# revollllt/FP8_quantization

Hardware: AMD Instinct MI355X
Metric: ImageNet val images/sec, ResNet-18 FP8 approx_v9 (higher is better)
Workload: dtype fp32; 1 GPU; resnet18 E4M3 approx_v9 forward (dnsmp_factor=3, withComp=False, with_s2nn2s_opt, quant_btw_mult_accu, res_quantizer, fixed ranges), ImageNet-shaped synthetic batch, random-init weights with BN statistics estimated on 4 synthetic batches; global_batch=1024, per_gpu_batch=1024, approx_macs_per_image=1814073344, parallelism=dp1

## Files before the change

### fp8_quantization_amd/_lib.py

```python
import ctypes
import os

import torch

HERE = os.path.dirname(os.path.abspath(__file__))
LIB_PATH = os.environ.get("FP8A_LIB_PATH") or os.path.join(HERE, "lib", "libfp8approx.so")

APPROX, S2N, QBMA, GCLIP, TB = 1, 2, 4, 8, 16
V5, OFUF, OF_OPT, UF_OPT = 32, 64, 128, 256
OK, EINVAL, EFORMAT, EHIP = 0, -1, -2, -3
DENSE_E4M3, DENSE_E5M2, DENSE_BF16 = 0, 1, 2

SYMBOLS = ("fp8a_version", "fp8a_last_error", "fp8a_fallback_stats", "fp8a_path_stats", "fp8a_kernel_timing", "fp8a_kernel_time", "fp8a_set_option", "fp8a_decompose", "fp8a_quant", "fp8a_matmul_workspace_size",
           "fp8a_matmul_workspace_size_mnk", "fp8a_matmul", "fp8a_terms", "fp8a_conv2d_workspace_size", "fp8a_conv2d",
           "fp8a_conv2d_bn_act", "fp8a_conv2d_qin_workspace_size", "fp8a_conv2d_qin",
           "fp8a_conv2d_block_workspace_size", "fp8a_conv2d_block", "fp8a_max_pool2d", "fp8a_avg_pool2d_plane", "fp8a_im2col",
           "fp8a_fp8_quantize", "fp8a_matmul_qamaa", "fp8a_conv2d_qamaa", "fp8a_matmul_block_workspace_size",
           "fp8a_matmul_block", "fp8a_dense_matmul_workspace_size", "fp8a_dense_matmul",
           "fp8a_dense_conv2d_workspace_size", "fp8a_dense_conv2d", "fp8a_grouped_conv2d", "fp8a_dense_conv2d_fused", "fp8a_dense_stats", "fp8a_clock_stats",
           "fp8a_word_image_bytes", "fp8a_word_image_init", "fp8a_conv2d_chain", "fp8a_conv2d_wants_image",
           "fp8a_flag_arena_slot_bytes")

_lib = None


class NativeLibraryMissing(RuntimeError):
    pass


def load():
    global _lib
    if _lib is not None:
        return _lib
    if not os.path.exists(LIB_PATH):
        raise NativeLibraryMissing(
            f"{LIB_PATH} not found: build it with `python -m fp8_quantization_amd.build_native` "
            "(there is no CPU fallback for the approx-FP8 path)")
    L = ctypes.CDLL(LIB_PATH)
    P, I, I64, U, SZ = ctypes.c_void_p, ctypes.c_int, ctypes.c_int64, ctypes.c_uint32, ctypes.c_size_t
    F = ctypes.c_float
    sig = {
        "fp8a_version": ([], ctypes.c_char_p),
        "fp8a_last_error": ([], ctypes.c_char_p),
        "fp8a_fallback_stats": ([P, I], I),
        "fp8a_path_stats": ([P, I], I),
        "fp8a_kernel_timing": ([I], I),
        "fp8a_kernel_time": ([P, I], I),
        "fp8a_set_option": ([ctypes.c_char_p, I], I),
        "fp8a_decompose": ([P, I64, I64, I64, I, I, P, I64, U, P, P, P], I),
        "fp8a_quant": ([P, I64, I, I, P, U, P, P], I),
        "fp8a_matmul_workspace_size": ([], SZ),
        "fp8a_matmul_workspace_size_mnk": ([I64, I64, I64], SZ),
        "fp8a_matmul": ([P, I64, P, I64, I64, P, I64, I64, I64, I64, I, I, P, P, I64, P, P, U, P, SZ, P], I),
        "fp8a_terms": ([P, I64, P, I64, I64, P, I64, I64, I64, I, I, P, P, I64, P, P, U, P], I),
        "fp8a_conv2d_workspace_size": ([I64, I64, I64, I64, I64, I, I, I, I, I, I, I, I, I], SZ),
        "fp8a_conv2d": ([P, P, P, I64, I64, I64, I64, I64, I, I, I, I, I, I, I, I, I, I, I, P, P, P, P, U, P, SZ, P],
                        I),
        "fp8a_conv2d_bn_act": ([P, P, P, I64, I64, I64, I64, I64, I, I, I, I, I, I, I, I, I, I, I, P, P, P, P, U, P,
                                I, F, F, P, SZ, P], I),
        "fp8a_conv2d_qin_workspace_size": ([I64, I64, I64, I64, I64, I, I, I, I, I, I, I, I, I], SZ),
        "fp8a_conv2d_qin": ([P, P, P, I64, I64, I64, I64, I64, I, I, I, I, I, I, I, I, I, I, I, P, P, P, U, P, I, F,
                             F, P, I, I, I, P, P, P, SZ, P], I),
        "fp8a_conv2d_block_workspace_size": ([I64, I64, I64, I64, I64, I, I, I, I, I, I, I, I, I], SZ),
        "fp8a_conv2d_block": ([P, P, P, I64, I64, I64, I64, I64, I, I, I, I, I, I, I, I, I, I, I, P, P, P, P, U, P, I,
                               F, F, P, I, I, I, P, P, P, I, F, F, P, I, I, I, P, P, P, SZ, P], I),
        "fp8a_word_image_bytes": ([I64, I64, I64, I64, I, I], SZ),
        "fp8a_word_image_init": ([P, I64, I64, I64, I64, I, I, P], I),
        "fp8a_conv2d_wants_image": ([I64, I, I, I, I, I, I, I, P, U, I, I, I, I], I),
        "fp8a_conv2d_chain": ([P, P, P, I64, I64, I64, I64, I64, I, I, I, I, I, I, I, I, I, I, I, P, P, P, P, U, P, I,
                               F, F, P, I, I, I, P, P, P, I, F, F, P, I, I, I, P, P, P, P, I, I, P, I, I, I, P, I,
                               I, P, SZ, P], I),
        "fp8a_max_pool2d": ([P, P, I64, I64, I64, I64, I, I, I, I, I, I, P], I),
        "fp8a_avg_pool2d_plane": ([P, P, I64, I64, I64, I64, I, I, I, I, P], I),
        "fp8a_im2col": ([P, P, I64, I64, I64, I64, I, I, I, I, I, I, I, I, P], I),
        "fp8a_fp8_quantize": ([P, I64, I64, P, I, I, I, I, P, P, P, P], I),
        "fp8a_matmul_qamaa": ([P, I64, P, I64, I64, P, I64, I64, I64, P, I, I, I, P], I),
        "fp8a_conv2d_qamaa": ([P, P, P, I64, I64, I64, I64, I64, I, I, I, I, I, I, I, I, I, P, I, I, I, P], I),
        "fp8a_matmul_block_workspace_size": ([I64, I64, I64], SZ),
        "fp8a_matmul_block": ([P, I64, P, I64, I64, P, I64, I64, I64, I64, I, I, P, P, I64, P, P, U, P, I, F, F, P, I, I,
                               I, P, P, P, I, F, F, P, I, I, I, P, P, P, SZ, P], I),
        "fp8a_dense_matmul_workspace_size": ([I64, I64, I64], SZ),
        "fp8a_dense_matmul": ([P, I64, I64, P, I64, I64, P, I64, I64, I64, I64, I, P, SZ, P], I),
        "fp8a_dense_conv2d_workspace_size": ([I64, I64, I64, I64, I64, I, I, I, I, I, I, I, I], SZ),
        "fp8a_dense_conv2d": ([P, P, P, I64, I64, I64, I64, I64, I, I, I, I, I, I, I, I, I, P, SZ, P], I),
        "fp8a_grouped_conv2d": ([P, P, P, I64, I64, I64, I64, I64, I, I, I, I, I, I, I, I, I, P], I),
        "fp8a_dense_conv2d_fused": ([P, P, P, I64, I64, I64, I64, I64, I, I, I, I, I, I, I, I, I, I,
                                     P, I, I, I, I, P, P, P, I, I, I, P, P, P, I, I, I, P, P, P, I, F, F,
                                     P, I, I, I, P, P, P, SZ, P], I),
        "fp8a_dense_stats": ([P, I], I),
        "fp8a_clock_stats": ([P, I], I),
        "fp8a_flag_arena_slot_bytes": ([P], SZ),
    }
    for name, (args, res) in sig.items():
        f = getattr(L, name)
        f.argtypes = args
        f.restype = res
    _lib = L
    return L


def version():
    return load().fp8a_version().decode()


def check(rc, what):
    if rc == OK:
        return
    msg = f"{what}: {load().fp8a_last_error().decode()}"
    if rc == EINVAL:
        raise AssertionError(msg)
    if rc == EFORMAT:
        raise ValueError(msg)
    raise RuntimeError(msg)


def stream_ptr(device):
    return ctypes.c_void_p(torch.cuda.current_stream(device).cuda_stream)


def dev_ptr(t):
    if t is None:
        return None
    if not t.is_cuda:
        raise RuntimeError("fp8approx kernels need HIP device tensors (no CPU fallback)")
    return ctypes.c_void_p(t.data_ptr())


def host_ptr(t):
    assert t.device.type == "cpu" and t.is_contiguous()
    return ctypes.c_void_p(t.data_ptr())


def flag_arena_slot_bytes(device=None):
    return int(load().fp8a_flag_arena_slot_bytes(stream_ptr(device)))


def fallback_stats(reset=False):
    L = load()
    out = (ctypes.c_uint64 * 4)()
    check(L.fp8a_fallback_stats(ctypes.cast(out, ctypes.c_void_p), 1 if reset else 0), "fp8a_fallback_stats")
    return dict(exact_launches=int(out[0]), exact_units=int(out[1]), f32_reruns=int(out[2]), tb_launches=int(out[3]))


PATHS = ("f8mx", "tt", "tt16", "fast", "exact", "dense", "v5mx")


def path_stats(reset=False):
    L = load()
    out = (ctypes.c_uint64 * len(PATHS))()
    check(L.fp8a_path_stats(ctypes.cast(out, ctypes.c_void_p), 1 if reset else 0), "fp8a_path_stats")
    return {k: int(v) for k, v in zip(PATHS, out)}


def kernel_timing(enable):
    return int(load().fp8a_kernel_timing(1 if enable else 0))


def kernel_time(reset=False):
    L = load()
    out = (ctypes.c_double * (4 * len(PATHS)))()
    check(L.fp8a_kernel_time(ctypes.cast(out, ctypes.c_void_p), 1 if reset else 0), "fp8a_kernel_time")
    return {k: dict(ms=out[4 * i], launches=int(out[4 * i + 1]), dispatches=int(out[4 * i + 2]), macs=out[4 * i + 3])
            for i, k in enumerate(PATHS) if out[4 * i + 1] > 0}


_option_gen = 0


def option_generation():
    return _option_gen


def set_option(name, value):
    global _option_gen
    rc = load().fp8a_set_option(name.encode(), int(value))
    if rc < 0:
        check(rc, "fp8a_set_option")
    _option_gen += 1
    return rc


def dense_stats(reset=False):
    L = load()
    out = (ctypes.c_uint64 * 2)()
    check(L.fp8a_dense_stats(ctypes.cast(out, ctypes.c_void_p), 1 if reset else 0), "fp8a_dense_stats")
    return dict(fp32_launches=int(out[0]), fp32_units=int(out[1]))


def clock_stats(reset=False):
    L = load()
    out = (ctypes.c_uint64 * 3)()
    check(L.fp8a_clock_stats(ctypes.cast(out, ctypes.c_void_p), 1 if reset else 0), "fp8a_clock_stats")
    t, r, n = int(out[0]), int(out[1]), int(out[2])
    return dict(memtime=t, realtime=r, workgroups=n, ghz=(t / r * 0.1) if r else None)
```

### fp8_quantization_amd/csrc/conv_tbx.h

```cpp
#pragma once
#include "fp8approx_common.h"
#include "gemm_dense.h"
#include "gemm_f8mx.h"

namespace fp8a {
constexpr int TBX_TW = 4;

struct TbxArgs {
    int64_t Cin, H, W, Cout, Ho, Wo;
    int kh, ph, pw, dh, cpg;
    uint32_t nwg, items;
};

__device__ __forceinline__ uint32_t tbx_word(float v, const FqIn &fq, float fmx, float fbias, uint32_t lowm,
                                             uint32_t mmask, int M, bool &bad) {
    if (fq.mx) v = fq_apply(v, fmx, fbias, fq.M, fq.S);
    const uint32_t u = __float_as_uint(v), ua = u & 0x7FFFFFFFu;
    bad |= (ua != 0u) && ((ua & lowm) != 0u || ua < 0x20800000u || ua > 0x58800000u);
    return ua == 0u ? 0u : ((u & 0xFF800000u) | (((ua >> (23 - M)) & mmask) << 3));
}

__global__ __launch_bounds__(256) void tbx_decode_a(const float *x, int64_t n, uint32_t *out, uint32_t *gate,
                                                    FqIn fq, float *fq_bias_out, int32_t *fq_ibias_out, int M = 3,
                                                    const uint32_t *img_hdr = nullptr) {
// ... 229 lines not shown
    float rv = e.x * __uint_as_float(cab);
    const float rs = copysignf(__fmaf_rn(2.0f, fabsf(rv), -twoq), rv);
    rv = ((__float_as_uint(rv) & 0x7F800000u) == q0exp) ? rs : rv;
    return (cab == __float_as_uint(e.y)) ? fabsf(rv) : rv;
}
template <int S, int M>
__global__ __launch_bounds__(256, TBSG_WAVES) void conv_tbsg_kernel(const float *x, const float *w, float *y, const DwArgs p,
                                                        FqIn fq, float *fq_bias_out, int32_t *fq_ibias_out,
                                                        const int32_t *bA, const int32_t *bW, const int32_t *bR,
                                                        TablePack tab, uint32_t *gate, const float2 *ep, int ep_act,
                                                        float ep_lo, float ep_hi, EmitW em) {
    constexpr int NC = 3 * S + 3;
    constexpr uint32_t LOWM = (1u << (23 - M)) - 1u, MMASK = (1u << M) - 1u;
    extern __shared__ float dw_sm[];
    const int tid = threadIdx.x, wv = tid >> 6;
    const int band = (int)(blockIdx.x % (unsigned)p.nb);
    const int64_t P0 = (int64_t)(blockIdx.x / (unsigned)p.nb) * p.PB;
    const int npl = (int)min((int64_t)p.PB, p.planes - P0);
    const int oh0 = band * p.RB, nrow = min(p.RB, p.Ho - oh0), hi0 = oh0 * S - p.ph;
    const int hw = p.H * p.W;
    const bool plane_mode = p.RB == p.Ho;
    const int rlo = plane_mode ? 0 : max(hi0, 0), rhi = plane_mode ? p.H : min(hi0 + p.RS, p.H);
    const int n = plane_mode ? npl * hw : (rhi - rlo) * p.W;
    const int64_t g0 = P0 * hw + (int64_t)rlo * p.W, a0 = g0 & ~(int64_t)3;
    const int lead = (int)(g0 - a0), nq = (lead + n + 3) >> 2;
    float2 *sL = reinterpret_cast<float2 *>(dw_sm);
    uint2 *sB = reinterpret_cast<uint2 *>(sL + 64);
    float2 *sT = reinterpret_cast<float2 *>(sB + 9 * p.PB);
    float *img = dw_sm + tbsg_img_off(p.PB);
    const float *src = x + a0;
    for (int q0 = 0; q0 < nq; q0 += 256) {
        const int q = q0 + tid;
        if (q < nq) {
            if (a0 + 4 * (int64_t)q + 4 <= p.nx) {
                __builtin_amdgcn_global_load_lds(src + 4 * q, img + 4 * (q0 + 64 * wv), 16, 0, 0);
            } else {
                for (int e = 0; e < 4; ++e)
                    if (a0 + 4 * (int64_t)q + e < p.nx) img[4 * q + e] = src[4 * q + e];
            }
        }
    }
    const float fmx = fq.mx ? *fq.mx : 0.0f, fbias = fq.mx ? fq_bias(fmx, fq.E, fq.M) : 0.0f;
    if (fq.mx && blockIdx.x == 0 && tid == 0) {
        *fq_bias_out = fbias;
        *fq_ibias_out = (int32_t)fbias;
    }
    const int a_b = fq.mx ? (int32_t)fbias : *bA, r_b = *bR;
    bool bad = !(a_b >= 2 && a_b <= 120 && r_b >= 2 && r_b <= 120);
    if (tid < 64) sL[tid] = tbx_lut_entry<M>(tid, tab, r_b);
    const int c0 = (int)(P0 % p.C);
    for (int d = tid; d < npl * 9; d += 256) {
        const int pl = d / 9;
        int c = c0 + pl;
        c -= dw_div(c, p.C, p.inv_c) * p.C;
        const int wb = bW[c];
        bad |= !(wb >= 2 && wb <= 120);
        const uint32_t bw = __float_as_uint(w[(int64_t)c * 9 + d - 9 * pl]), bwa = bw & 0x7FFFFFFFu;
        bad |= (bwa != 0u) && ((bwa & LOWM) != 0u || bwa < 0x20800000u || bwa > 0x58800000u);
        sB[d] = make_uint2(bw & 0xFF800000u, ((bwa >> (23 - M)) & MMASK) << 6);
    }
    __syncthreads();
    uint32_t *iw = reinterpret_cast<uint32_t *>(img);
    {
        const int i0 = lead, i1 = lead + n;
        for (int i = i0 + tid; i < i1; i += 256) iw[i] = tbx_word(img[i], fq, fmx, fbias, LOWM, MMASK, M, bad);
    }
    if (TBSG_TAPT) {
        for (int e = tid; e < npl * 72; e += 256) {
            const uint2 b = sB[e >> 3];
            const float2 l = sL[(b.y >> 3) + (e & 7)];
            const uint32_t t = __float_as_uint(l.y), cb = b.x;
            const int ef = (int)((t >> 23) & 0xFFu) - (int)((cb >> 23) & 0xFFu) + 127;
            const bool ok = t != 0xFFFFFFFFu && (cb & 0x7F800000u) != 0u && ef >= 1 && ef <= 254;
            const uint32_t tq = ok ? (((t ^ cb) & 0x80000000u) | ((uint32_t)ef << 23)) : 0xFFFFFFFFu;
            sT[e] = make_float2(l.x * __uint_as_float(cb), __uint_as_float(tq));
        }
    }
    __syncthreads();
    const uint32_t q0exp = (uint32_t)(127 - r_b) << 23;
    const float twoq = __uint_as_float((uint32_t)(128 - r_b) << 23);
    const char *lut = reinterpret_cast<const char *>(sL);
    const int nqd = (p.Wo + 3) >> 2, pq = p.RB * nqd;
    float emx = 0.0f, efb = 0.0f;
    uint32_t eemn = 0u, sehi = 0u;
    int ebR = 0;
    bool eok = true;
    if (em.w) {
        emx = __uint_as_float(__builtin_amdgcn_readfirstlane((int)em.invalid[1]));
        efb = __uint_as_float(__builtin_amdgcn_readfirstlane((int)em.invalid[2]));
        eemn = __builtin_amdgcn_readfirstlane(em.invalid[3]);
        ebR = __builtin_amdgcn_readfirstlane((int)em.invalid[4]);
    }
    for (int e = tid; e < npl * pq; e += 256) {
        const int pl = dw_div(e, pq, p.inv_pq), rem = e - pl * pq;
        const int orow = dw_div(rem, nqd, p.inv_nqd), qd = rem - orow * nqd;
        if (orow >= nrow) continue;
        const int r0 = (oh0 + orow) * S - p.ph, cl = 4 * S * qd - p.pw;
        const uint32_t *xs = iw + lead + pl * hw + (r0 - rlo) * p.W + cl;
        const uint2 *wb = sB + pl * 9;
        bool cok[NC];
#pragma unroll
        for (int c = 0; c < NC; ++c) cok[c] = (unsigned)(cl + c) < (unsigned)p.W;
        float acc[4] = {0.0f, 0.0f, 0.0f, 0.0f};
#pragma unroll TBSG_KYU
        for (int ky = 0; ky < 3; ++ky) {
            const bool rok = (unsigned)(r0 + ky) < (unsigned)p.H;
            uint32_t col[NC];
#pragma unroll
            for (int c = 0; c < NC; ++c) col[c] = (rok && cok[c]) ? xs[ky * p.W + c] : 0u;
#pragma unroll
            for (int kx = 0; kx < 3; ++kx) {
                if (TBSG_TAPT) {
                    const char *tap = reinterpret_cast<const char *>(sT + 8 * (9 * pl + 3 * ky + kx));
#pragma unroll
                    for (int j = 0; j < 4; ++j) acc[j] += tbx_term_t(col[j * S + kx], tap, q0exp, twoq);
                } else {
                    const uint2 b = wb[3 * ky + kx];
                    const float cB = __uint_as_float(b.x);
#pragma unroll
                    for (int j = 0; j < 4; ++j) acc[j] += tbx_term(col[j * S + kx], cB, b.y, lut, q0exp, twoq);
                }
            }
        }
        int co = c0 + pl;
        co -= dw_div(co, p.C, p.inv_c) * p.C;
        float *yo = y + ((P0 + pl) * p.Ho + oh0 + orow) * p.Wo + 4 * qd;
        uint32_t *wo = em.w ? em.w + ((uint32_t)(P0 + pl) * (uint32_t)em.awH + (uint32_t)(oh0 + orow + em.awph)) *
                                         (uint32_t)em.awW + (uint32_t)em.awpw + 4u * (uint32_t)qd
                            : nullptr;
#pragma unroll
        for (int j = 0; j < 4; ++j)
            if (4 * qd + j < p.Wo) {
                const float o = epi(ep, ep_act, ep_lo, ep_hi, co, acc[j]);
                yo[j] = o;
                if (wo) {
                    const uint32_t wd = xm_word_a(fq_apply(o, emx, efb, em.fq.M, em.fq.S), em.Mw, xm_xbias(em.Mw), eemn,
                                                  ebR, eok);
                    wo[j] = wd;
                    sehi = max(sehi, word_sehi(wd));
                }
            }
    }
    if (em.w) wave_max_atomic(em.invalid + 5, sehi);
    const bool ebad = em.w && !eok;
    if (__syncthreads_or(bad ? 1 : 0) && tid == 0) {
        atomicOr(gate, 1u);
        if (em.w) atomicOr(em.invalid, 1u);
    }
    if (__syncthreads_or(ebad ? 1 : 0) && tid == 0) atomicOr(em.invalid, 1u);
}


__global__ __launch_bounds__(256) void v5dw_decode_a(const float *x, int64_t n, uint32_t *out, int E, int M,
                                                     const int32_t *bA, FqIn fq, float *fqb, int32_t *fqi) {
    const float fmx = fq.mx ? *fq.mx : 0.0f, fbias = fq.mx ? fq_bias(fmx, fq.E, fq.M) : 0.0f;
    if (fq.mx && blockIdx.x == 0 && threadIdx.x == 0) {
        *fqb = fbias;
        *fqi = (int32_t)fbias;
    }
    const DFmt f = dfmt(E, M, fq.mx ? (int)fbias : *bA, false);
    for (int64_t i = (int64_t)blockIdx.x * blockDim.x + threadIdx.x; i < n; i += (int64_t)gridDim.x * blockDim.x) {
        float v = x[i];
        if (fq.mx) v = fq_apply(v, fmx, fbias, fq.M, fq.S);
        int e, m;
        exact_dec(v, f, true, e, m);
        out[i] = (v < 0.0f ? 0x80000000u : 0u) | ((uint32_t)(m * 8) << 16) | (uint32_t)(e * (1 << M) + m);
    }
}

__global__ __launch_bounds__(256) void v5dw_decode_b(const float *w, int64_t n, int taps, uint2 *out, int E, int M,
                                                     const int32_t *bA, const int32_t *bW, const int32_t *bR,
                                                     TablePack tab) {
    const int a_b = *bA, r_b = *bR;
    for (int64_t i = (int64_t)blockIdx.x * blockDim.x + threadIdx.x; i < n; i += (int64_t)gridDim.x * blockDim.x) {
        const int64_t co = i / taps;
        const int b_b = bW[co];
        const float v = w[i];
        int e, m;
        exact_dec(v, dfmt(E, M, b_b, false), true, e, m);
        const int32_t cb = (e - (a_b + b_b - r_b)) * (1 << M) + m;
        uint32_t row = 0;
        for (int ma = 0; ma < 4; ++ma) row |= ((uint32_t)(uint8_t)tab.raw[(ma << M) | m]) << (8 * ma);
        out[i] = make_uint2(((uint32_t)cb << 1) | (v < 0.0f ? 1u : 0u), row);
    }
}

template <int SW>
__global__ __launch_bounds__(256) void conv_v5dw_kernel(const uint32_t *aw, const uint2 *bw, float *y, TbxArgs t,
                                                        const int32_t *bR, uint32_t flags, int E, uint32_t *gate,
                                                        const float2 *ep,
                                                        int ep_act, float ep_lo, float ep_hi) {
    constexpr int KW = 3, NCOL = (TBX_TW - 1) * SW + KW, M = 2;
    const int r_b = *bR;
    const int32_t maxi = ((1 << E) << M) - 1;
    bool bad = !(r_b >= -90 && r_b <= 120);
    const uint32_t lin0 = (uint32_t)(127 - r_b) << 23;
    const float csub = __uint_as_float((uint32_t)(126 - r_b) << 23);
    const int64_t HW = t.H * t.W;
    for (uint32_t item = blockIdx.x * blockDim.x + threadIdx.x; item < t.items; item += gridDim.x * blockDim.x) {
        const uint32_t wg = item % t.nwg, r1 = item / t.nwg;
        const uint32_t ho = r1 % (uint32_t)t.Ho, r2 = r1 / (uint32_t)t.Ho;
        const uint32_t co = r2 % (uint32_t)t.Cout, img = r2 / (uint32_t)t.Cout;
        const int wo0 = (int)wg * TBX_TW, wi0 = wo0 * SW - t.pw;
        float acc[TBX_TW] = {0.0f, 0.0f, 0.0f, 0.0f};
        const uint32_t *plane = aw + ((int64_t)img * t.Cin + (int64_t)co) * HW;
        const uint2 *wk = bw + (int64_t)co * t.kh * KW;
        for (int ky = 0; ky < t.kh; ++ky) {
            const int hi = (int)ho * SW - t.ph + ky * t.dh;
            const bool rowok = (uint32_t)hi < (uint32_t)t.H;
            const uint32_t *row = plane + (int64_t)hi * t.W;
            uint32_t col[NCOL];
#pragma unroll
            for (int j = 0; j < NCOL; ++j) {
                const int wi = wi0 + j;
                col[j] = (rowok && (uint32_t)wi < (uint32_t)t.W) ? row[wi] : 0u;
            }
#pragma unroll
            for (int kx = 0; kx < KW; ++kx) {
                const uint2 b = wk[ky * KW + kx];
                const int32_t cb = (int32_t)b.x >> 1;
                const uint32_t sb = b.x << 31;
#pragma unroll
                for (int q = 0; q < TBX_TW; ++q) {
                    const uint32_t wa = col[q * SW + kx];
                    const int32_t tv = __builtin_amdgcn_sbfe((int32_t)b.y, (wa >> 16) & 31u, 8);
                    int32_t r = (int32_t)(wa & 0xFFu) + cb + tv;
// ... 151 lines not shown
```

### fp8_quantization_amd/csrc/fp8approx.hip

```cpp
#include <hip/hip_runtime.h>
#include <stdint.h>
#include <string.h>

#include <algorithm>
#include <atomic>
#include <cmath>
#include <cstdlib>
#include <cstdio>
#include <map>
#include <mutex>
#include <string>
#include <vector>

#include "../../include/fp8approx.h"
#include "fp8approx_common.h"
#include "fp8approx_launch.h"
#include "gemm_f8mx.h"
#include "gemm_v5mx.h"
#include "gemm_tt.h"
#include "gemm_tt16.h"
#include "gemm_dense.h"
#include "conv_tbx.h"

extern "C" __global__ void fq_bias_kernel(fp8a::FqIn fq, float *bias_out, int32_t *ibias_out);

namespace fp8a {

static thread_local std::string g_err;

static int fail(int code, const std::string &msg) {
    g_err = msg;
    return code;
}

static int hip_check(const char *what) {
    hipError_t e = hipGetLastError();
    if (e != hipSuccess) return fail(FP8A_EHIP, std::string(what) + ": " + hipGetErrorString(e));
    return FP8A_OK;
}

static int pack_table(const int32_t *table, int M, bool approx, TablePack &tp, int &mode) {
    memset(&tp, 0, sizeof(tp));
    mode = TM_NONE;
    if (!approx || table == nullptr) return FP8A_OK;
    const int n = 1 << M;
    if (n * n > 1024) return fail(FP8A_EFORMAT, "error table larger than 32x32 (mant_width > 5)");
    int lo = 0, hi = 0;
    for (int i = 0; i < n * n; ++i) {
        if (table[i] < -128 || table[i] > 127) return fail(FP8A_EINVAL, "error table entry out of int8 range");
        tp.raw[i] = (int8_t)table[i];
        lo = std::min(lo, table[i]);
        hi = std::max(hi, table[i]);
    }
    if (lo == 0 && hi == 0) return FP8A_OK;
    const int words2 = (n * 2 + 31) / 32;
    if (lo >= 0 && hi <= 1 && n <= 32) {
        mode = TM_W1U;
        for (int i = 0; i < n; ++i)
            for (int j = 0; j < n; ++j)
                if (table[i * n + j]) tp.rows[i][0] |= 1u << j;
    } else if (lo >= -2 && hi <= 1 && words2 <= 2) {
        mode = words2 == 1 ? TM_W2S1 : TM_W2S2;
    } else if (lo >= 0 && hi <= 3 && words2 <= 2) {
        mode = words2 == 1 ? TM_W2U1 : TM_W2U2;
    } else {
        mode = TM_LUT;
    }
    if (mode >= TM_W2S1 && mode <= TM_W2U2) {
        for (int i = 0; i < n; ++i)
            for (int j = 0; j < n; ++j) {
                const uint32_t code = (uint32_t)table[i * n + j] & 3u;
                const int bit = j * 2;
                tp.rows[i][bit >> 5] |= code << (bit & 31);
            }
    }
    return FP8A_OK;
}

__device__ unsigned long long g_fallback[4];

__global__ __launch_bounds__(256) void splitk_reduce_kernel(const GemmArgs p) {
    const int64_t MN = p.M * p.N;
    const float pb = post_bias(p);
    const EmitCtx ec = emit_ctx(p);
    uint32_t sehi = 0;
    const int S = p.splits;
    const bool vec = p.nchw ? ((p.hw & 3) == 0) : ((p.N & 3) == 0 && (p.ldc & 3) == 0);
    const bool aligned = ((((uintptr_t)p.C) & 15) == 0) && ((((uintptr_t)p.part) & 15) == 0) && ((MN & 3) == 0) &&
                         ((((uintptr_t)p.res) & 15) == 0);
    const int64_t stride = (int64_t)gridDim.x * blockDim.x;
    if (vec && aligned) {
        for (int64_t q4 = (int64_t)blockIdx.x * blockDim.x + threadIdx.x; q4 < MN / 4; q4 += stride) {
            const int64_t q = q4 * 4;
            float4 acc = *reinterpret_cast<const float4 *>(p.part + q);
            for (int sp = 1; sp < S; ++sp) {
                const float4 v = *reinterpret_cast<const float4 *>(p.part + sp * MN + q);
                acc.x += v.x; acc.y += v.y; acc.z += v.z; acc.w += v.w;
            }
            int64_t o;
            if (p.nchw) {
                const int64_t img = q / (p.N * p.hw), rem = q - img * p.N * p.hw, n = rem / p.hw, pix = rem - n * p.hw;
                o = (img * p.ctot + p.coff + n) * p.hw + pix;
                if (p.ep) {
                    const int64_t ch = p.coff + n;
                    acc.x = epi(p.ep, p.ep_act, p.ep_lo, p.ep_hi, ch, acc.x);
                    acc.y = epi(p.ep, p.ep_act, p.ep_lo, p.ep_hi, ch, acc.y);
                    acc.z = epi(p.ep, p.ep_act, p.ep_lo, p.ep_hi, ch, acc.z);
                    acc.w = epi(p.ep, p.ep_act, p.ep_lo, p.ep_hi, ch, acc.w);
                }
            } else {
                const int64_t m = q / p.N, n = q - m * p.N;
                o = m * p.ldc + n;
                if (p.ep) {
                    acc.x = epi(p.ep, p.ep_act, p.ep_lo, p.ep_hi, p.coff + n, acc.x);
                    acc.y = epi(p.ep, p.ep_act, p.ep_lo, p.ep_hi, p.coff + n + 1, acc.y);
                    acc.z = epi(p.ep, p.ep_act, p.ep_lo, p.ep_hi, p.coff + n + 2, acc.z);
                    acc.w = epi(p.ep, p.ep_act, p.ep_lo, p.ep_hi, p.coff + n + 3, acc.w);
                }
            }
            const float4 r = post4(p, o, acc, pb);
            *reinterpret_cast<float4 *>(p.C + o) = r;
            if (p.em.w) emit4(p, ec, o, r, sehi);
        }
        if (p.em.w) wave_max_atomic(p.em.invalid + 5, sehi);
        return;
    }
    for (int64_t q = (int64_t)blockIdx.x * blockDim.x + threadIdx.x; q < MN; q += stride) {
        float acc = p.part[q];
        for (int sp = 1; sp < S; ++sp) acc += p.part[sp * MN + q];
        int64_t o, ch;
        if (p.nchw) {
            const int64_t img = q / (p.N * p.hw), rem = q - img * p.N * p.hw, n = rem / p.hw, pix = rem - n * p.hw;
            o = (img * p.ctot + p.coff + n) * p.hw + pix;
            ch = p.coff + n;
        } else {
            const int64_t m = q / p.N, n = q - m * p.N;
            o = m * p.ldc + n;
            ch = p.coff + n;
        }
        const float r = post1(p, o, epi(p.ep, p.ep_act, p.ep_lo, p.ep_hi, ch, acc), pb);
        p.C[o] = r;
        if (p.em.w) emit1(p, ec, o, r, sehi);
    }
    if (p.em.w) wave_max_atomic(p.em.invalid + 5, sehi);
}

__device__ __forceinline__ float load_A(const GemmArgs &p, int64_t m, int64_t k) {
    if (!p.conv) {
        const float v = p.A[m * p.lda + k];
        if (p.fqin.mx == nullptr) return v;
        const float mx = *p.fqin.mx;
        return fq_apply(v, mx, fq_bias(mx, p.fqin.E, p.fqin.M), p.fqin.M, p.fqin.S);
    }
    const int64_t hw = p.Ho * p.Wo, img = m / hw, pix = m - img * hw;
    const int64_t ho = pix / p.Wo, wo = pix - ho * p.Wo;
    const int64_t taps = (int64_t)p.kh * p.kw, c = k / taps, t = k - c * taps, ky = t / p.kw, kx = t - ky * p.kw;
    const int64_t hi = ho * p.sh - p.ph + ky * p.dh, wi = wo * p.sw - p.pw + kx * p.dw;
    if (hi < 0 || hi >= p.H || wi < 0 || wi >= p.W) return 0.0f;
    const float v = p.X[((img * p.Cin + p.cbase + c) * p.H + hi) * p.W + wi];
    if (p.fqin.mx == nullptr) return v;
    const float mx = *p.fqin.mx;
    return fq_apply(v, mx, fq_bias(mx, p.fqin.E, p.fqin.M), p.fqin.M, p.fqin.S);
}

__device__ __forceinline__ void gemm_exact_units(const GemmArgs &p, uint32_t f, const DFmt &fA, const DFmt &fR, bool tb);

__global__ __launch_bounds__(256) void gemm_exact_kernel(const GemmArgs p) {
    const bool tb = p.flags & F_TB;
    if (p.post_bout != nullptr && blockIdx.x == 0 && threadIdx.x == 0) {
        const float b = fq_bias(*p.post_fq.mx, p.post_fq.E, p.post_fq.M);
        *p.post_bout = b;
        *p.post_ibout = (int32_t)b;
    }
    const DFmt fA = dfmt(p.E, p.Mw, *p.bA, tb), fR = dfmt(p.E, p.Mw, *p.bR, tb);
    if (p.flag == nullptr) {
        for (int64_t idx = (int64_t)blockIdx.x * blockDim.x + threadIdx.x; idx < p.M * p.N;
             idx += (int64_t)gridDim.x * blockDim.x) {
            const int64_t m = idx % p.M, n = idx / p.M;
            const DFmt fB = dfmt(p.E, p.Mw, p.bB[n * p.bBs], tb);
            float s = 0.0f, part = 0.0f;
            for (int64_t k = 0; k < p.K; ++k) {
                part += exact_term(load_A(p, m, k), p.B[k * p.sbk + n * p.sbn], fA, fB, fR, p.tab.raw, p.flags);
                if ((k & 15) == 15) {
                    s += part;
                    part = 0.0f;
                }
            }
            s += part;
            const int64_t o = out_index(p, m, n);
            const float r = post1(p, o, epi(p.ep, p.ep_act, p.ep_lo, p.ep_hi, p.coff + n, s), post_bias(p));
            p.C[o] = r;
            if (p.em.w) {
                uint32_t sh = 0;
                emit1(p, emit_ctx(p), o, r, sh);
                if (sh) atomicMax(p.em.invalid + 5, sh);
            }
        }
        return;
    }
    arena_clear(p.arena_clr, p.arena_clr16);
    const uint32_t f = __hip_atomic_load(p.flag, __ATOMIC_RELAXED, __HIP_MEMORY_SCOPE_AGENT);
    if (p.flag_out && blockIdx.x == 0 && threadIdx.x == 0) *p.flag_out = f;
    if (f & FB_ANY) gemm_exact_units(p, f, fA, fR, tb);
}

__device__ __forceinline__ void gemm_exact_units(const GemmArgs &p, uint32_t f, const DFmt &fA, const DFmt &fR, bool tb) {
    const bool all = (f & FB_ALL) != 0u || p.urow == nullptr;
    const int64_t nur = (p.M + 63) >> 6, nuc = (p.N + 63) >> 6;
    if (blockIdx.x == 0 && threadIdx.x == 0) atomicAdd(&g_fallback[0], 1ull);
    const float pb = post_bias(p);
    const EmitCtx ec = emit_ctx(p);
    for (int64_t u = blockIdx.x; u < nur * nuc; u += gridDim.x) {
        const int64_t ur = u / nuc, uc = u - ur * nuc;
        if (!all && !p.urow[ur] && !p.ucol[uc] && !(p.utile[u] & UT_EXACT)) continue;
        if (threadIdx.x == 0) atomicAdd(&g_fallback[1], 1ull);
        const int64_t m = 64 * ur + (threadIdx.x & 63), nb = 64 * uc + 16 * (threadIdx.x >> 6);
        if (m >= p.M) continue;
        float s[16], part[16];
        DFmt fB[16];
#pragma unroll
        for (int j = 0; j < 16; ++j) {
            s[j] = part[j] = 0.0f;
            fB[j] = dfmt(p.E, p.Mw, p.bB[min(nb + j, p.N - 1) * p.bBs], tb);
        }
        for (int64_t k = 0; k < p.K; ++k) {
            const float a = load_A(p, m, k);
#pragma unroll
            for (int j = 0; j < 16; ++j) {
                const int64_t n = min(nb + j, p.N - 1);
                part[j] += exact_term(a, p.B[k * p.sbk + n * p.sbn], fA, fB[j], fR, p.tab.raw, p.flags);
                if ((k & 15) == 15) {
                    s[j] += part[j];
                    part[j] = 0.0f;
                }
            }
        }
#pragma unroll
        for (int j = 0; j < 16; ++j) {
            const int64_t n = nb + j;
            if (n >= p.N) break;
            const int64_t o = out_index(p, m, n);
            const float r = post1(p, o, epi(p.ep, p.ep_act, p.ep_lo, p.ep_hi, p.coff + n, s[j] + part[j]), pb);
            p.C[o] = r;
            if (p.em.w) {
                uint32_t sh = 0;
                emit1(p, ec, o, r, sh);
                if (sh) atomicMax(p.em.invalid + 5, sh);
            }
        }
    }
}

__global__ __launch_bounds__(256) void terms_kernel(const GemmArgs p, float *T) {
    const int64_t idx = (int64_t)blockIdx.x * blockDim.x + threadIdx.x;
    if (idx >= p.M * p.K * p.N) return;
    const int64_t n = idx % p.N, k = (idx / p.N) % p.K, m = idx / (p.N * p.K);
    const bool tb = p.flags & F_TB;
    const DFmt fA = dfmt(p.E, p.Mw, *p.bA, tb), fR = dfmt(p.E, p.Mw, *p.bR, tb);
    const DFmt fB = dfmt(p.E, p.Mw, p.bB[n * p.bBs], tb);
    T[idx] = exact_term(p.A[m * p.lda + k], p.B[k * p.sbk + n * p.sbn], fA, fB, fR, p.tab.raw, p.flags);
}

__global__ __launch_bounds__(256) void decompose_kernel(const float *x, int64_t rows, int64_t cols, int64_t ld,
                                                        int E, int M, const int32_t *bias, int64_t bs,
                                                        uint32_t flags, int32_t *expo, int32_t *mant) {
    const int64_t idx = (int64_t)blockIdx.x * blockDim.x + threadIdx.x;
    if (idx >= rows * cols) return;
    const int64_t r = idx / cols, c = idx - r * cols;
    const DFmt f = dfmt(E, M, bias[r * bs], flags & F_TB);
    int e, m;
    exact_dec(x[r * ld + c], f, flags & F_GCLIP, e, m);
    expo[idx] = e;
    mant[idx] = m;
}

__global__ __launch_bounds__(256) void quant_kernel(const float *x, int64_t n, int E, int M, const int32_t *bias,
                                                    uint32_t flags, float *out) {
    const int64_t idx = (int64_t)blockIdx.x * blockDim.x + threadIdx.x;
    if (idx >= n) return;
    const DFmt f = dfmt(E, M, *bias, flags & F_TB);
    out[idx] = exact_q(x[idx], f, flags & F_GCLIP);
}

__global__ __launch_bounds__(256) void im2col_kernel(const float *x, float *out, int64_t Bn, int64_t C, int64_t H,
                                                     int64_t W, int kh, int kw, int sh, int sw, int ph, int pw,
                                                     int dh, int dw, int64_t Ho, int64_t Wo) {
    const int64_t K = C * kh * kw;
    const int64_t total = Bn * Ho * Wo * K;
    for (int64_t idx = (int64_t)blockIdx.x * blockDim.x + threadIdx.x; idx < total;
         idx += (int64_t)gridDim.x * blockDim.x) {
        const int64_t k = idx % K, m = idx / K;
        const int64_t kx = k % kw, ky = (k / kw) % kh, c = k / (kw * kh);
        const int64_t wo = m % Wo, ho = (m / Wo) % Ho, b = m / (Wo * Ho);
        const int64_t hi = ho * sh - ph + ky * dh, wi = wo * sw - pw + kx * dw;
        float v = 0.0f;
        if (hi >= 0 && hi < H && wi >= 0 && wi < W) v = x[((b * C + c) * H + hi) * W + wi];
        out[idx] = v;
    }
}

template <bool TB>
__global__ __launch_bounds__(256) void conv_tb_direct_kernel(const float *x, const float *w, float *y, int64_t Bn,
                                                             int64_t Cin, int64_t H, int64_t W, int64_t Cout,
                                                             int kh, int kw, int sh, int sw, int ph, int pw, int dh,
                                                             int dw, int groups, int64_t Ho, int64_t Wo, int E,
                                                             int Mw, const int32_t *bA, const int32_t *bW,
                                                             const int32_t *bR, TablePack tab, uint32_t flags,
                                                             const uint32_t *gate, uint32_t *gate_out, uint4 *clr,
                                                             uint32_t clr16, const float2 *ep, int ep_act,
                                                             float ep_lo, float ep_hi, FqIn fq) {
    arena_clear(clr, clr16);
    const uint32_t gv = gate != nullptr ? __hip_atomic_load(gate, __ATOMIC_RELAXED, __HIP_MEMORY_SCOPE_AGENT) : 1u;
    if (gate_out != nullptr && blockIdx.x == 0 && threadIdx.x == 0) *gate_out = gv;
    if (gv == 0u) return;
    if (gate != nullptr && blockIdx.x == 0 && threadIdx.x == 0) atomicAdd(&g_fallback[3], 1ull);
    const int64_t total = Bn * Cout * Ho * Wo;
    const int64_t cpg = Cin / groups;
    const DFmt fA = dfmt(E, Mw, *bA, TB), fR = dfmt(E, Mw, *bR, TB);
    const float fmx = fq.mx ? *fq.mx : 0.0f, fbias = fq.mx ? fq_bias(fmx, fq.E, fq.M) : 0.0f;
    for (int64_t idx = (int64_t)blockIdx.x * blockDim.x + threadIdx.x; idx < total;
         idx += (int64_t)gridDim.x * blockDim.x) {
        const int64_t wo = idx % Wo, ho = (idx / Wo) % Ho, co = (idx / (Wo * Ho)) % Cout, b = idx / (Wo * Ho * Cout);
        const int64_t g = co / (Cout / groups);
        const DFmt fB = dfmt(E, Mw, bW[co], TB);
        float s = 0.0f, part = 0.0f;
        int cnt = 0;
        for (int64_t c = 0; c < cpg; ++c)
            for (int ky = 0; ky < kh; ++ky)
                for (int kx = 0; kx < kw; ++kx) {
                    const int64_t hi = ho * sh - ph + ky * dh, wi = wo * sw - pw + kx * dw;
// ... 126 lines not shown
                const int wi = w0 + kx;
                if ((unsigned)wi >= (unsigned)W) continue;
                const float v = xp[(int64_t)hi * W + wi];
                m = (v > m || v != v) ? v : m;
            }
        }
        y[idx] = m;
    }
}

__global__ __launch_bounds__(128) void avg_pool_plane_kernel(const float *x, float *y, int64_t planes, int PB, int W,
                                                             int hw, int ps, int kh, int kw, float inv_hw) {
    extern __shared__ float ap_sm[];
    const int tid = threadIdx.x;
    const int64_t P0 = (int64_t)blockIdx.x * PB;
    const int npl = (int)min((int64_t)PB, planes - P0), n = npl * hw;
    const float *xb = x + P0 * hw;
    for (int d0 = tid; d0 < n; d0 += 4 * 128) {
        float v[4];
#pragma unroll
        for (int u = 0; u < 4; ++u) v[u] = d0 + 128 * u < n ? xb[d0 + 128 * u] : 0.0f;
#pragma unroll
        for (int u = 0; u < 4; ++u) {
            const int d = d0 + 128 * u;
            if (d < n) {
                const int pl = dw_div(d, hw, inv_hw);
                ap_sm[pl * ps + d - pl * hw] = v[u];
            }
        }
    }
    __syncthreads();
    for (int t = tid; t < npl; t += 128) {
        const float *s = ap_sm + t * ps;
        float acc = 0.0f;
        for (int r = 0; r < kh; ++r)
            for (int c = 0; c < kw; ++c) acc += s[r * W + c];
        y[P0 + t] = acc / (float)(kh * kw);
    }
}

__global__ __launch_bounds__(256) void max_pool2d_s2k3_kernel(const float *x, float *y, int64_t planes, int H, int W,
                                                             int Ho) {
    const int Wq = W / 8;
    const int64_t total = planes * Ho * Wq;
    for (int64_t idx = (int64_t)blockIdx.x * blockDim.x + threadIdx.x; idx < total;
         idx += (int64_t)gridDim.x * blockDim.x) {
        const int q = (int)(idx % Wq);
        const int64_t t = idx / Wq;
        const int ho = (int)(t % Ho);
        const int64_t pl = t / Ho;
        const float *xp = x + pl * H * W;
        float m[4] = {-INFINITY, -INFINITY, -INFINITY, -INFINITY};
        const int c0 = 8 * q;
#pragma unroll
        for (int ky = 0; ky < 3; ++ky) {
            const int hi = 2 * ho - 1 + ky;
            if ((unsigned)hi >= (unsigned)H) continue;
            const float *r = xp + (int64_t)hi * W + c0;
            const float4 a = *reinterpret_cast<const float4 *>(r), b = *reinterpret_cast<const float4 *>(r + 4);
            const float v[9] = {c0 > 0 ? r[-1] : -INFINITY, a.x, a.y, a.z, a.w, b.x, b.y, b.z, b.w};
#pragma unroll
            for (int o = 0; o < 4; ++o)
#pragma unroll
                for (int kx = 0; kx < 3; ++kx) {
                    if (o == 0 && kx == 0 && c0 == 0) continue;
                    const float u = v[2 * o + kx];
                    m[o] = (u > m[o] || u != u) ? u : m[o];
                }
        }
        *reinterpret_cast<float4 *>(y + (pl * Ho + ho) * (int64_t)(W / 2) + 4 * q) = make_float4(m[0], m[1], m[2], m[3]);
    }
}

static void launch_f8mx(const GemmArgs &a, hipStream_t s) {
    if (a.Mw == 2) {
        launch_f8mx_xf1(a, s);
        launch_f8mx_xf2(a, s);
    } else {
        launch_f8mx_xf0(a, s);
    }
}

static int g_opt_xm_ncg = getenv("FP8A_XM_NCG") ? atoi(getenv("FP8A_XM_NCG")) : 0;
static int xm_ncg(int64_t N) {
    const int forced = g_opt_xm_ncg;
    if (forced == 1 || forced == 2 || forced == 4) return forced;
    int best = 4;
    int64_t bp = (N + 63) / 64 * 64;
    for (int c : {2, 1}) {
        const int64_t pad = (N + 16 * c - 1) / (16 * c) * (16 * c);
        if (pad < bp) {
            bp = pad;
            best = c;
        }
    }
    return best;
}

static void launch_fast(int mode, const GemmArgs &a, hipStream_t s) {
    const int64_t tiles = ((a.M + BM - 1) / BM) * ((a.N + BN - 1) / BN);
    const dim3 grid((unsigned)(tiles * a.splits));
    if (mode == TM_V5) {
        if (a.aw && a.wfmt == 4) launch_v5mx(a, s);
        else launch_fast_p0(TM_V5, false, a, grid, s);
        return;
    }
    if (mode == TM_QAMAA) {
        launch_fast_p0(TM_QAMAA, false, a, grid, s);
        return;
    }
    if (a.aw && (a.wfmt == 1 || a.wfmt == 2)) {
        launch_tt(a, grid, s);
        return;
    }
    if (mode == TM_F8) {
        if (a.aw || a.af32) launch_f8mx(a, s);
        else launch_fast_p3(TM_F8, false, a, grid, s);
        return;
    }
    const bool s2n = a.flags & F_S2N, q = a.flags & F_QBMA, gc = a.flags & F_GCLIP;
    if (s2n) q ? launch_fast_p3(mode, gc, a, grid, s) : launch_fast_p2(mode, gc, a, grid, s);
    else q ? launch_fast_p1(mode, gc, a, grid, s) : launch_fast_p0(mode, gc, a, grid, s);
}

static int check_format(int E, int Mw) {
    if (E < 1 || Mw < 1 || Mw > 5 || E > 6 || E + Mw > 8)
        return fail(FP8A_EFORMAT, "Invalid combination of expo_width and mant_width");
    return FP8A_OK;
}

constexpr size_t FLAG_BYTES = 256;

enum { PATH_F8MX = 0, PATH_TT = 1, PATH_TT16 = 2, PATH_FAST = 3, PATH_EXACT = 4, PATH_DENSE = 5, PATH_V5MX = 6,
       PATH_N = 7 };
static std::atomic<uint64_t> g_paths[PATH_N];

struct KernelEv {
    hipEvent_t a, b;
    int path, dispatches;
    double macs;
};
static bool g_ktime = false;
static std::vector<KernelEv> g_kev;
static std::vector<hipEvent_t> g_evpool;
static hipEvent_t pool_event() {
    if (!g_evpool.empty()) {
        hipEvent_t e = g_evpool.back();
        g_evpool.pop_back();
        return e;
    }
    hipEvent_t e = nullptr;
    if (hipEventCreate(&e) != hipSuccess) {
        (void)hipGetLastError();
        return nullptr;
    }
    return e;
}
static int g_opt_tbx_rw = getenv("FP8A_TBX_RW") ? atoi(getenv("FP8A_TBX_RW")) : 2;
static int g_opt_tbs = getenv("FP8A_TBS") ? atoi(getenv("FP8A_TBS")) : 2;
static int g_opt_dw3 = getenv("FP8A_DW3") ? atoi(getenv("FP8A_DW3")) : 2;
static int g_opt_dn_direct = getenv("FP8A_DN_DIRECT") ? atoi(getenv("FP8A_DN_DIRECT")) : 1;
static int g_opt_v5ds = getenv("FP8A_V5DS") ? atoi(getenv("FP8A_V5DS")) : 1;
static int g_opt_dw_target = getenv("FP8A_DW_TARGET") ? atoi(getenv("FP8A_DW_TARGET")) : 4096;
static int g_opt_dw_lds = getenv("FP8A_DW_LDS") ? atoi(getenv("FP8A_DW_LDS")) : 40960;

static int device_cus() {
    static int cache[64] = {0};
    int dev = 0;
    if (hipGetDevice(&dev) != hipSuccess || dev < 0 || dev >= 64) {
        (void)hipGetLastError();
        return 256;
    }
    if (cache[dev] == 0) {
        int cus = 0;
        if (hipDeviceGetAttribute(&cus, hipDeviceAttributeMultiprocessorCount, dev) != hipSuccess || cus <= 0) {
            (void)hipGetLastError();
            cus = 256;
        }
        cache[dev] = cus;
    }
    return cache[dev];
}

static int choose_splits(int64_t M, int64_t N, int64_t K) {
    static int forced = -1;
    if (forced < 0) {
        const char *e = getenv("FP8A_SPLITK");
        forced = e ? std::max(0, atoi(e)) : 0;
    }
    const int64_t kt = (K + BK - 1) / BK;
    if (forced > 0) return (int)std::max<int64_t>(1, std::min<int64_t>(forced, kt));
    const int64_t tiles = ((M + BM - 1) / BM) * ((N + BN - 1) / BN);
    const double slots = 4.0 * device_cus();
    static double rate = 0.0;
    if (rate == 0.0) {
        const char *e = getenv("FP8A_SPLITK_RATE");
        rate = e ? std::max(1e8, atof(e)) : 4.4e9;
    }
    const double t_round = (double)BM * BN * K / rate;
    const double t_split = 2.0 * (double)M * N * sizeof(float) / 2.0e12;
    double best = 1e300;
    int bs = 1;
    for (int S = 1; S <= 8; ++S) {
        if (S > 1 && kt < 16 * S) break;
        const double q = (double)tiles * S / slots, fl = std::floor(q), fr = q - fl;
        const double rounds = fl + (fr > 1e-9 ? std::min(1.0, 0.4 + 1.1 * fr) : 0.0);
        const double t = rounds / S * t_round + (S > 1 ? S * t_split : 0.0);
        if (t < best * (1.0 - 1e-3)) {
            best = t;
            bs = S;
        }
    }
    return bs;
}

static size_t align256(size_t x) { return (x + 255) & ~(size_t)255; }

static size_t xm_b_bytes(int64_t kpad, int64_t npad) { return align256((size_t)(kpad * npad) * 8); }
static size_t xm_operand_bytes(int64_t N, int64_t K, int64_t a_words) {
    const int64_t kpad = (K + BK - 1) / BK * BK, npad = (N + BN - 1) / BN * BN;
    return align256((size_t)a_words * 4) + xm_b_bytes(kpad, npad) + 16384 + align256((size_t)(kpad * npad / 16) * 2);
}

static size_t unit_bytes(int64_t M, int64_t N) {
    const int64_t nur = (M + 63) / 64, nuc = (N + 63) / 64;
    return align256((size_t)(nur + nuc + nur * nuc));
}
static size_t head_bytes(int64_t M, int64_t N) { return FLAG_BYTES + unit_bytes(M, N); }

static size_t splitk_bytes(int64_t M, int64_t N, int64_t K) {
    const int S = choose_splits(M, N, K);
    return S > 1 ? align256((size_t)S * (size_t)M * (size_t)N * sizeof(float)) : 0;
}


static size_t gemm_workspace_bytes(int64_t M, int64_t N, int64_t K, int64_t conv_words) {
    const int64_t a_words = conv_words > 0 ? conv_words : M * ((K + BK - 1) / BK * BK);
    return head_bytes(M, N) + splitk_bytes(M, N, K) + xm_operand_bytes(N, K, a_words);
}

static bool f8_form(int E, int Mw, uint32_t flags, int table_mode) {
    static const bool no_f8 = getenv("FP8A_NO_F8") != nullptr;
    static const bool no_f8_e5 = getenv("FP8A_NO_F8_E5M2") != nullptr;
    const bool fmt = (E == 4 && Mw == 3) || (E == 5 && Mw == 2 && !no_f8_e5);
    return !no_f8 && !(flags & F_V5) && fmt && (table_mode == TM_NONE || table_mode == TM_W1U) &&
           (flags & F_S2N) && (flags & F_QBMA) && !(flags & F_GCLIP) && !(flags & F_TB);
}

static bool v5mx_form(int Mw, uint32_t flags, int table_mode) {
    static const bool no_v5mx = getenv("FP8A_NO_V5MX") != nullptr;
    return table_mode == TM_V5 && Mw == 2 && (flags & F_OFUF) && !no_v5mx;
}

static bool tt_form(int Mw, uint32_t flags, const TablePack &tab) {
    static const bool no_tt = getenv("FP8A_NO_TT") != nullptr;
    if (no_tt || (flags & F_V5) || !(Mw == 4 || Mw == 5) || !(flags & F_S2N) || !(flags & F_QBMA) ||
        (flags & F_GCLIP) || (flags & F_TB))
        return false;
    bool neg = false;
    for (int i = 0; i < (1 << (2 * Mw)); ++i) neg |= tab.raw[i] < 0;
    return Mw == 4 || !neg;
}

static int g_opt_tt16_mink = getenv("FP8A_TT16_MINK") ? std::max(0, atoi(getenv("FP8A_TT16_MINK"))) : 64;
static int g_opt_tt_band = getenv("FP8A_TT_BAND") ? atoi(getenv("FP8A_TT_BAND")) : 1;
static bool tt16_form(int Mw, bool f7, int64_t K) {
// ... 144 lines not shown
static int run_qamaa(GemmArgs &a, hipStream_t s);

static int run_gemm(GemmArgs &a, const int32_t *table, void *ws, size_t ws_bytes, hipStream_t s) {
    if (a.qmax) return run_qamaa(a, s);
    int rc = check_format(a.E, a.Mw);
    if (rc) return rc;
    if (a.M < 0 || a.N < 0 || a.K < 0) return fail(FP8A_EINVAL, "negative extent");
    if (a.post_bout && (a.M == 0 || a.N == 0 || a.K == 0)) {
        fq_bias_kernel<<<1, 1, 0, s>>>(a.post_fq, a.post_bout, a.post_ibout);
        const int rc0 = hip_check("fp8a output-quantizer bias");
        if (rc0) return rc0;
    }
    if (a.M == 0 || a.N == 0) return FP8A_OK;
    if (a.K == 0) {
        if (a.nchw) return fail(FP8A_EINVAL, "empty convolution window");
        if (dev_zero_rows(a.C, a.ldc, a.N, a.M, s) != hipSuccess)
            return hip_check("fp8a zero fill");
        return FP8A_OK;
    }
    if ((!a.A && !a.conv) || (a.conv && !a.X) || !a.B || !a.C || !a.bA || !a.bB || !a.bR)
        return fail(FP8A_EINVAL, "null pointer");
    int mode;
    const bool v5 = a.flags & F_V5;
    if (v5 && (a.flags & F_TB)) return fail(FP8A_EINVAL, "the v5 model has no tensor-bias semantics");
    rc = pack_table(table, a.Mw, v5 || (a.flags & F_APPROX), a.tab, mode);
    if (rc) return rc;
    if (v5) mode = TM_V5;
    const int mode0 = mode;
    if (f8_form(a.E, a.Mw, a.flags, mode)) mode = TM_F8;
    const int64_t total = a.M * a.N;
    const unsigned eblocks = (unsigned)std::min<int64_t>((total + 255) / 256, 4096);
    if (a.flags & F_TB) {
        a.flag = nullptr;
        ++g_paths[PATH_EXACT];
        gemm_exact_kernel<<<eblocks, 256, 0, s>>>(a);
        return hip_check("fp8a exact gemm launch");
    }
    if (ws == nullptr || ws_bytes < FLAG_BYTES) return fail(FP8A_EINVAL, "matmul workspace too small");
    static const bool no_units = getenv("FP8A_NO_UNITS") != nullptr;
    const size_t head = ws_bytes >= head_bytes(a.M, a.N) ? head_bytes(a.M, a.N) : FLAG_BYTES;
    ArenaLease lease;
    const int cap = stream_capturing(s);
    if (cap < 0) return hip_check("fp8a stream capture query");
    if (cap ? !capture_lease(s, ws, ws_bytes, head, lease) : !flag_arena(s, head_bytes(a.M, a.N), lease))
        return lease_error();
    a.flag = lease.mine;
    a.flag_out = (uint32_t *)ws;
    a.arena_clr = lease.clr;
    a.arena_clr16 = lease.clr16;
    a.nur = (a.M + 63) / 64;
    a.nuc = (a.N + 63) / 64;
    a.urow = no_units || (cap && head < head_bytes(a.M, a.N)) ? nullptr : (uint8_t *)a.flag + FLAG_BYTES;
    a.ucol = no_units ? nullptr : a.urow + a.nur;
    a.utile = no_units ? nullptr : a.ucol + a.nuc;
    a.splits = choose_splits(a.M, a.N, a.K);
    if (a.splits > 1 && ws_bytes < head + splitk_bytes(a.M, a.N, a.K)) a.splits = 1;
    const int64_t kt = (a.K + BK - 1) / BK;
    a.kchunk = ((kt + a.splits - 1) / a.splits) * BK;
    a.part = a.splits > 1 ? (float *)((char *)ws + head) : nullptr;
    a.aw = nullptr;
    const bool tt = mode != TM_F8 && tt_form(a.Mw, a.flags, a.tab);
    const bool v5mx = v5mx_form(a.Mw, a.flags, mode);
    if ((mode == TM_F8 || tt || v5mx) && !no_mx()) {
        const int64_t kpad = kt * BK, npad = (a.N + BN - 1) / BN * BN;
        const size_t off = head + (a.splits > 1 ? splitk_bytes(a.M, a.N, a.K) : 0);
        const int64_t a_words = xm_a_words(a);
        const WordImage wi = word_image(a.H, a.W, a.ph, a.pw);
        a.awH = wi.H; a.awW = wi.W; a.awph = wi.ph; a.awpw = wi.pw;
        const bool fits32 = a_words < (1ll << 30) && kpad * npad * 4 < (1ll << 32);
        if (fits32 && ws_bytes >= off + xm_operand_bytes(a.N, a.K, a_words)) {
            char *base = (char *)ws + off;
            a.aw = (const uint32_t *)base;
            a.awld = kpad;
            a.bqw = (const uint2 *)(base + align256((size_t)a_words * 4));
            a.lutw = (const uint32_t *)(base + align256((size_t)a_words * 4) + xm_b_bytes(kpad, npad));
            a.ebr = (const uint16_t *)((const char *)a.lutw + 16384);
            a.xm_vmin = mode == TM_NONE ? 0 : -1;
            a.npad = npad;
            a.ttf7 = 0;
            for (int i = 0; tt && i < (1 << (2 * a.Mw)); ++i) a.ttf7 |= a.tab.raw[i] < 0;
            a.wfmt = v5mx ? 4 : tt ? (tt16_form(a.Mw, a.ttf7, a.K) ? 2 : 1) : 0;
            if (a.wfmt == 1 && !g_opt_tt_band) a.ebr = nullptr;
            a.xncg = tt ? 4 : xm_ncg(a.N);
            const bool use_img = a.in_img != nullptr && !tt && a.conv && a.fqin.mx != nullptr;
            if (use_img) a.aw = a.in_img + 64;
            a.af32 = !tt && !v5mx && !use_img && xm_af32(a) ? 1 : 0;
            const int64_t rows = a.conv ? a.M / (a.Ho * a.Wo) : a.M, cols = a_words / std::max<int64_t>(rows, 1);
            dim3 ga((unsigned)std::min<int64_t>((cols + 255) / 256, 64), (unsigned)std::min<int64_t>(rows, 1024));
            {
                const int64_t hw = a.H * a.W, lim0 = a.conv ? cols : a.K, istride = a.conv ? a.Cin * hw : a.lda;
                const float *in0 = a.conv ? a.X + a.cbase * hw : a.A;
                const bool flat = !(a.conv && (a.awph | a.awpw)) && lim0 % 4 == 0 && cols % 4 == 0 && istride % 4 == 0 &&
                                  ((uintptr_t)in0 & 15) == 0 && ((uintptr_t)a.aw & 15) == 0;
                if (flat) ga = dim3((unsigned)std::max<int64_t>(1, std::min<int64_t>((a_words / 4 + 1023) / 1024, 8192)), 1);
            }
            if (use_img) {
                a.gate = a.in_img;
                xm_decode_a<<<ga.y == 1 ? dim3(std::min(ga.x, 512u)) : dim3(std::min(ga.x, 8u), std::min(ga.y, 64u)), 256, 0,
                              s>>>(a);
                a.gate = nullptr;
            } else if (!a.af32) {
                xm_decode_a<<<ga, 256, 0, s>>>(a);
            }
            if (v5mx) {
                const unsigned gb = (unsigned)std::min<int64_t>((kpad * npad + 255) / 256, 4096);
                v5mx_decode_b<<<gb, 256, 0, s>>>(a, kpad);
            } else if (tt) {
                const unsigned gb = (unsigned)std::min<int64_t>((kpad * npad + 255) / 256, 4096);
                tt_decode_b<<<gb, 256, 0, s>>>(a, kpad);
            } else {
                const unsigned gb = (unsigned)std::min<int64_t>((kpad * npad / 2 + 255) / 256, 4096);
                xm_decode_b<<<gb, 256, 0, s>>>(a, kpad);
            }
            rc = hip_check("fp8a operand pre-decode launch");
            if (rc) return rc;
        }
    }
    if (a.fqin.mx && !a.aw)
        return fail(FP8A_EINVAL, "internal: fused input quantization without the matrix-core path");
    if (mode == TM_F8 && a.Mw != 3 && !a.aw) mode = mode0;
    ++g_paths[!a.aw ? PATH_FAST : a.wfmt == 0 ? PATH_F8MX : a.wfmt == 1 ? PATH_TT : a.wfmt == 4 ? PATH_V5MX : PATH_TT16];
    if (a.em.w != nullptr && (a.em.form == 2 || (a.aw && a.wfmt != 0 && a.splits == 1) || a.post_act == 2)) {
        if (dev_fill(a.em.invalid, 1, sizeof(uint32_t), s) != hipSuccess) return hip_check("fp8a word image header");
        a.em.w = nullptr;
    }
    KernelEv kev{};
    if (g_ktime && !cap) {
        kev.a = pool_event();
        kev.b = pool_event();
        kev.path = !a.aw ? PATH_FAST : a.wfmt == 0 ? PATH_F8MX : a.wfmt == 1 ? PATH_TT : a.wfmt == 4 ? PATH_V5MX : PATH_TT16;
        kev.dispatches = (a.aw && ((a.wfmt == 0 && a.Mw == 2) || a.wfmt == 2)) ? 2 : 1;
        kev.macs = (double)a.M * (double)a.N * (double)a.K;
        if (kev.a && kev.b) (void)hipEventRecord(kev.a, s);
    }
    launch_fast(mode, a, s);
    if (g_ktime && !cap && kev.a && kev.b) {
        (void)hipEventRecord(kev.b, s);
        g_kev.push_back(kev);
    }
    rc = hip_check("fp8a fast gemm launch");
    if (rc) return rc;
    if (a.splits > 1) {
        const int64_t q = a.M * a.N;
        const unsigned rb = (unsigned)std::min<int64_t>((q / 4 + 255) / 256 + 1, 8192);
        splitk_reduce_kernel<<<rb, 256, 0, s>>>(a);
        rc = hip_check("fp8a split-K reduce launch");
        if (rc) return rc;
    }
    const unsigned ublocks = std::max((unsigned)std::min<int64_t>(a.nur * a.nuc, 512), clear_blocks(lease));
    gemm_exact_kernel<<<ublocks, 256, 0, s>>>(a);
    rc = hip_check("fp8a gated exact gemm launch");
    static const bool dbg = getenv("FP8A_DEBUG_FLAGS") != nullptr;
    if (!rc && dbg) {
        uint32_t f = 0;
        if (hipStreamSynchronize(s) == hipSuccess && hipMemcpy(&f, a.flag_out, sizeof(f), hipMemcpyDeviceToHost) == hipSuccess)
            fprintf(stderr, "fp8a flag M=%lld N=%lld K=%lld E=%d M=%d wfmt=%d flag=%u\n", (long long)a.M, (long long)a.N,
                    (long long)a.K, a.E, a.Mw, a.aw ? a.wfmt : -1, f);
    }
    return rc;
}

static int run_qamaa(GemmArgs &a, hipStream_t s) {
    if (a.M < 0 || a.N < 0 || a.K < 0) return fail(FP8A_EINVAL, "negative extent");
    if (a.M == 0 || a.N == 0) return FP8A_OK;
    if (a.qM < 1 || a.qE < 1) return fail(FP8A_EFORMAT, "bad qamaa quantizer format");
    if (!a.nchw && a.ldc != a.N) return fail(FP8A_EINVAL, "qamaa output must be dense");
    if (a.K == 0) {
        if (dev_fill(a.C, 0, (size_t)a.M * a.N * sizeof(float), s) != hipSuccess) return hip_check("fill");
    } else {
        a.splits = 1;
        a.kchunk = a.K;
        launch_fast(TM_QAMAA, a, s);
        int rc = hip_check("fp8a qamaa gemm launch");
        if (rc) return rc;
    }
    return FP8A_OK;
}

static inline int64_t round_up(int64_t v, int64_t m) { return (v + m - 1) / m * m; }
static inline size_t al256(size_t b) { return (b + 255) & ~(size_t)255; }

static size_t dense_ws_bytes(int64_t M, int64_t N, int64_t K) {
    const int64_t mpad = round_up(std::max<int64_t>(M, 1), DN_T), npad = round_up(std::max<int64_t>(N, 1), DN_T);
    const int64_t kpad = round_up(std::max<int64_t>(K, 1), 32);
    return al256(4 * (size_t)(mpad / DN_U + npad / DN_U) + 4) + al256((size_t)(2 * mpad * kpad)) +
           al256((size_t)(mpad * kpad / 32)) + al256((size_t)(2 * npad * kpad)) + al256((size_t)(npad * kpad / 32));
}

static uint32_t next_dense_gen() {
    static std::atomic<uint32_t> ctr{0};
    uint32_t g;
    do {
        g = (ctr.fetch_add(1) + 1) * 0x9E3779B1u;
        g ^= g >> 15;
    } while (g == 0u);
    return g;
}

static int run_dense(DenseArgs a, void *ws, size_t wsb, hipStream_t s) {
    if (a.M < 0 || a.N < 0 || a.K < 0) return fail(FP8A_EINVAL, "negative extent");
    if (a.fmt != FP8A_DENSE_E4M3 && a.fmt != FP8A_DENSE_E5M2 && a.fmt != FP8A_DENSE_BF16)
        return fail(FP8A_EINVAL, "unknown dense operand format");
    const bool qout = a.fz.qin.mx || a.fz.rq.mx || a.fz.oq.mx || a.fz.wq.mx;
    if (qout && (a.M == 0 || a.K == 0)) {
        dn_bias_kernel<<<(unsigned)std::max<int64_t>(1, (a.N + 255) / 256), 256, 0, s>>>(a.fz, a.N);
        const int rc = hip_check("fp8a dense quantizer biases");
        if (rc) return rc;
    }
    if (a.M == 0 || a.N == 0) return FP8A_OK;
    ++g_paths[PATH_DENSE];
    if (a.K == 0) {
        const hipError_t e = a.conv ? dev_fill(a.y, 0, (size_t)(a.M * a.N) * sizeof(float), s)
                                    : dev_zero_rows(a.y, a.ldc, a.N, a.M, s);
        return e == hipSuccess ? FP8A_OK : hip_check("fp8a dense fill");
    }
    if (g_opt_dn_direct && a.conv && a.K <= DD_K && a.N <= DD_N) {
        KernelEv kev{};
        if (g_ktime) {
            kev.a = pool_event();
            kev.b = pool_event();
            kev.path = PATH_DENSE;
            kev.dispatches = 1;
            kev.macs = 4.0 * ((double)a.M * a.K + (double)a.M * a.N) + 4.0 * (double)a.N * a.K;
            if (kev.a && kev.b) (void)hipEventRecord(kev.a, s);
        }
        const unsigned g = (unsigned)std::min<int64_t>((a.M + 255) / 256, 1 << 20);
        dn_direct_kernel<<<g, 256, 0, s>>>(a);
        if (g_ktime && kev.a && kev.b) {
// ... 124 lines not shown
    if (H >= (1 << 20) || W >= (1 << 20) || C >= (1 << 20) || H * W >= (1ll << 22)) return false;
    a.planes = planes; a.C = (int)C; a.H = (int)H; a.W = (int)W; a.Ho = (int)Ho; a.Wo = (int)Wo; a.ph = ph; a.pw = pw;
    const int nq = (int)((Wo + TBX_TW - 1) / TBX_TW);
    const int WS = ((4 * nq - 1) * S + 3 + 3) / 4 * 4;
    const int64_t op = Ho * Wo;
    for (int target = std::max(256, g_opt_dw_target); target >= 256; target /= 2) {
        int PB, RB;
        if (op <= target) {
            RB = (int)Ho;
            PB = (int)std::min<int64_t>(target / op, planes);
            if (H * W % 4 != 0 && PB >= 4) PB &= ~3;
        } else {
            PB = 1;
            RB = std::max(1, (int)(target / Wo));
        }
        const int RS = (RB - 1) * S + 3;
        const int64_t bytes = (int64_t)PB * RS * WS * 4 + 512 + (int64_t)PB * 9 * 8;
        if (bytes > std::min(65536, std::max(4096, g_opt_dw_lds))) continue;
        a.PB = PB; a.RB = RB; a.nb = (int)((Ho + RB - 1) / RB); a.RS = RS; a.WS = WS; a.nq = nq;
        a.inv_c = 1.0f / a.C; a.inv_ws = 1.0f / WS; a.inv_pst = 1.0f / (RS * WS);
        a.inv_nq = 1.0f / nq; a.inv_pq = 1.0f / (RB * nq);
        a.inv_w = 1.0f / a.W; a.inv_hw = 1.0f / (a.H * a.W);
        lds = (size_t)bytes;
        return ((planes + PB - 1) / PB) * a.nb < (1ll << 24);
    }
    return false;
}

extern "C" {

const char *fp8a_version(void) { return "fp8approx gfx950 r1"; }

const char *fp8a_last_error(void) { return g_err.c_str(); }

int fp8a_path_stats(uint64_t *out, int reset) {
    if (out == nullptr) return fail(FP8A_EINVAL, "null pointer");
    for (int i = 0; i < PATH_N; ++i) out[i] = reset ? g_paths[i].exchange(0) : g_paths[i].load();
    return FP8A_OK;
}

size_t fp8a_flag_arena_slot_bytes(fp8a_stream_t stream) {
    int dev = 0;
    if (hipGetDevice(&dev) != hipSuccess) return 0;
    std::lock_guard<std::mutex> lock(g_arena_mu);
    const auto it = g_arenas.find({dev, (uintptr_t)stream});
    return it == g_arenas.end() ? 0 : it->second.slot;
}

int fp8a_kernel_timing(int enable) {
    const int old = g_ktime ? 1 : 0;
    g_ktime = enable != 0;
    return old;
}

int fp8a_kernel_time(double *out, int reset) {
    if (out == nullptr) return fail(FP8A_EINVAL, "null pointer");
    for (int i = 0; i < 4 * PATH_N; ++i) out[i] = 0.0;
    for (const KernelEv &e : g_kev) {
        if (hipEventSynchronize(e.b) != hipSuccess) return hip_check("fp8a_kernel_time");
        float ms = 0.0f;
        if (hipEventElapsedTime(&ms, e.a, e.b) != hipSuccess) return hip_check("fp8a_kernel_time");
        out[4 * e.path] += ms;
        out[4 * e.path + 1] += 1.0;
        out[4 * e.path + 2] += e.dispatches;
        out[4 * e.path + 3] += e.macs;
    }
    if (reset) {
        for (const KernelEv &e : g_kev) {
            g_evpool.push_back(e.a);
            g_evpool.push_back(e.b);
        }
        g_kev.clear();
    }
    return FP8A_OK;
}

int fp8a_set_option(const char *name, int value) {
    if (name == nullptr) return fail(FP8A_EINVAL, "null pointer");
    if (strcmp(name, "xm_ncg") == 0) {
        const int old = g_opt_xm_ncg;
        g_opt_xm_ncg = value;
        return old;
    }
    if (strcmp(name, "af32_maxct") == 0) {
        const int old = g_opt_af32_maxct;
        g_opt_af32_maxct = std::max(0, value);
        return old;
    }
    if (strcmp(name, "tt_band") == 0) {
        const int old = g_opt_tt_band;
        g_opt_tt_band = value;
        return old;
    }
    if (strcmp(name, "tt16_mink") == 0) {
        const int old = g_opt_tt16_mink;
        g_opt_tt16_mink = std::max(0, value);
        return old;
    }
    if (strcmp(name, "tbx_rw") == 0) {
        const int old = g_opt_tbx_rw;
        g_opt_tbx_rw = value;
        return old;
    }
    if (strcmp(name, "tbs") == 0) {
        const int old = g_opt_tbs;
        g_opt_tbs = value;
        return old;
    }
    if (strcmp(name, "dw_lds") == 0) {
        const int old = g_opt_dw_lds;
        g_opt_dw_lds = std::min(65536, std::max(4096, value));
        return old;
    }
    if (strcmp(name, "dw_target") == 0) {
        const int old = g_opt_dw_target;
        g_opt_dw_target = std::max(256, value);
        return old;
    }
    if (strcmp(name, "dn_direct") == 0) {
        const int old = g_opt_dn_direct;
        g_opt_dn_direct = value;
        return old;
    }
    if (strcmp(name, "v5ds") == 0) {
        const int old = g_opt_v5ds;
        g_opt_v5ds = value;
        return old;
    }
    if (strcmp(name, "dw3") == 0) {
        const int old = g_opt_dw3;
        g_opt_dw3 = value;
        return old;
    }
    return fail(FP8A_EINVAL, std::string("unknown option ") + name);
}

int fp8a_fallback_stats(uint64_t *out, int reset) {
    if (out == nullptr) return fail(FP8A_EINVAL, "null pointer");
    unsigned long long v[4] = {0, 0, 0, 0}, tt = 0;
    if (hipDeviceSynchronize() != hipSuccess || hipMemcpyFromSymbol(v, HIP_SYMBOL(g_fallback), sizeof(v)) != hipSuccess ||
        tt_rerun_stats(&tt, reset != 0) != 0)
        return hip_check("fp8a_fallback_stats");
    for (int i = 0; i < 4; ++i) out[i] = v[i];
    out[2] = tt;
    if (reset) {
        const unsigned long long z[4] = {0, 0, 0, 0};
        if (hipMemcpyToSymbol(HIP_SYMBOL(g_fallback), z, sizeof(z)) != hipSuccess) return hip_check("fp8a_fallback_stats");
    }
    return FP8A_OK;
}

size_t fp8a_dense_matmul_workspace_size(int64_t M, int64_t N, int64_t K) { return dense_ws_bytes(M, N, K); }

int fp8a_dense_matmul(const float *A, int64_t sam, int64_t sak, const float *B, int64_t sbk, int64_t sbn, float *C,
                      int64_t ldc, int64_t M, int64_t N, int64_t K, int fmt, void *workspace, size_t workspace_bytes,
                      fp8a_stream_t stream) {
    if (ldc < N) return fail(FP8A_EINVAL, "leading dimension smaller than extent");
    DenseArgs a = dense_args();
    a.x = A; a.sam = sam; a.sak = sak; a.w = B; a.sbk = sbk; a.sbn = sbn; a.y = C; a.ldc = ldc;
    a.M = M; a.N = N; a.K = K; a.fmt = fmt;
    return run_dense(a, workspace, workspace_bytes, (hipStream_t)stream);
}

size_t fp8a_dense_conv2d_workspace_size(int64_t Bn, int64_t Cin, int64_t H, int64_t W, int64_t Cout, int kh, int kw,
                                        int sh, int sw, int ph, int pw, int dh, int dw) {
    const int64_t Ho = (H + 2 * ph - dh * (kh - 1) - 1) / sh + 1;
// ... 11 lines not shown
    const int64_t Wo = (W + 2 * pw - dw * (kw - 1) - 1) / sw + 1;
    if (Ho <= 0 || Wo <= 0) return fail(FP8A_EINVAL, "empty convolution output");
    DenseArgs a = dense_args();
    a.x = x; a.w = w; a.y = y; a.conv = 1;
    a.C = Cin; a.H = H; a.W = W; a.Ho = Ho; a.Wo = Wo;
    a.kh = kh; a.kw = kw; a.sh = sh; a.sw = sw; a.ph = ph; a.pw = pw; a.dh = dh; a.dw = dw;
    a.M = Bn * Ho * Wo; a.N = Cout; a.K = Cin * kh * kw;
    a.sbk = 1; a.sbn = a.K;
    a.ldc = Cout; a.fmt = fmt;
    return run_dense(a, workspace, workspace_bytes, (hipStream_t)stream);
}

static int grouped_conv_impl(const float *x, const float *w, float *y, int64_t Bn, int64_t Cin, int64_t H, int64_t W,
                             int64_t Cout, int groups, int kh, int kw, int sh, int sw, int ph, int pw, int dh, int dw,
                             const DnFuse &fz, hipStream_t stream);

int fp8a_grouped_conv2d(const float *x, const float *w, float *y, int64_t Bn, int64_t Cin, int64_t H, int64_t W,
                        int64_t Cout, int groups, int kh, int kw, int sh, int sw, int ph, int pw, int dh, int dw,
                        fp8a_stream_t stream) {
    return grouped_conv_impl(x, w, y, Bn, Cin, H, W, Cout, groups, kh, kw, sh, sw, ph, pw, dh, dw, DnFuse{},
                             (hipStream_t)stream);
}

static int grouped_conv_impl(const float *x, const float *w, float *y, int64_t Bn, int64_t Cin, int64_t H, int64_t W,
                             int64_t Cout, int groups, int kh, int kw, int sh, int sw, int ph, int pw, int dh, int dw,
                             const DnFuse &fz, hipStream_t stream) {
    if (kh < 1 || kw < 1 || sh < 1 || sw < 1 || dh < 1 || dw < 1 || ph < 0 || pw < 0 || Bn < 0 || Cin < 0 || Cout < 0)
        return fail(FP8A_EINVAL, "bad convolution geometry");
    if (groups < 1 || Cin % groups != 0 || Cout % groups != 0) return fail(FP8A_EINVAL, "channels not divisible by groups");
    const int64_t Ho = (H + 2 * ph - dh * (kh - 1) - 1) / sh + 1;
    const int64_t Wo = (W + 2 * pw - dw * (kw - 1) - 1) / sw + 1;
    if (Ho <= 0 || Wo <= 0) return fail(FP8A_EINVAL, "empty convolution output");
    GcArgs a{};
    a.x = x; a.w = w; a.y = y;
    a.Cin = Cin; a.H = H; a.W = W; a.Cout = Cout; a.Ho = Ho; a.Wo = Wo;
    a.total = Bn * Cout * Ho * ((Wo + GC_OW - 1) / GC_OW);
    a.cig = (int)(Cin / groups); a.cog = (int)(Cout / groups);
    a.kh = kh; a.kw = kw; a.sh = sh; a.sw = sw; a.ph = ph; a.pw = pw; a.dh = dh; a.dw = dw;
    a.fz = fz;
    if (a.total == 0) {
        if (fz.qin.mx || fz.rq.mx || fz.oq.mx || fz.wq.mx) {
            dn_bias_kernel<<<(unsigned)std::max<int64_t>(1, (Cout + 255) / 256), 256, 0, stream>>>(fz, Cout);
            return hip_check("fp8a grouped conv quantizer biases");
        }
        return FP8A_OK;
    }
    if (!x || !w || !y) return fail(FP8A_EINVAL, "null pointer");
    if (g_opt_dw3 && a.cig == 1 && a.cog == 1 && kh == 3 && kw == 3 && dh == 1 && dw == 1 && sh == sw && pw <= DW_OX &&
        (sh == 1 || sh == 2)) {
        DwArgs d{};
        d.x = x; d.w = w; d.y = y; d.fz = fz;
        d.planes = Bn * Cout; d.C = (int)Cout; d.H = (int)H; d.W = (int)W; d.Ho = (int)Ho; d.Wo = (int)Wo;
        d.ph = ph; d.pw = pw;
        size_t lds = 0;
        d.nx = Bn * Cin * H * W;
        const bool raw = g_opt_dw3 == 2;
        if (H < (1 << 20) && W < (1 << 20) && Cout < (1 << 20) && H * W < (1ll << 22) && plan_dw3(d, sh, lds, raw)) {
            const unsigned g = (unsigned)(((d.planes + d.PB - 1) / d.PB) * d.nb);
            if (raw && sh == 1) dn_dw3g_kernel<1><<<g, 256, lds, stream>>>(d);
            else if (raw) dn_dw3g_kernel<2><<<g, 256, lds, stream>>>(d);
            else if (sh == 1) dn_dw3_kernel<1><<<g, 256, lds, stream>>>(d);
            else dn_dw3_kernel<2><<<g, 256, lds, stream>>>(d);
            ++g_paths[PATH_DENSE];
            return hip_check("fp8a depthwise conv launch");
        }
    }
    if (a.total + 65536ll * 256 < (1ll << 31)) launch_group_conv<uint32_t>(a, stream);
    else launch_group_conv<int64_t>(a, stream);
    ++g_paths[PATH_DENSE];
    return hip_check("fp8a grouped conv launch");
}

int fp8a_clock_stats(uint64_t *out, int reset) {
    if (out == nullptr) return fail(FP8A_EINVAL, "null pointer");
    if (hipDeviceSynchronize() != hipSuccess) return hip_check("fp8a_clock_stats");
    unsigned long long v[3] = {0, 0, 0};
    int (*parts[3])(unsigned long long *, bool) = {f8mx_clock_xf0, f8mx_clock_xf1, f8mx_clock_xf2};
    for (auto f : parts) {
        unsigned long long w[3] = {0, 0, 0};
        if (f(w, reset != 0) != 0) return hip_check("fp8a_clock_stats");
        for (int i = 0; i < 3; ++i) v[i] += w[i];
    }
    for (int i = 0; i < 3; ++i) out[i] = v[i];
    return FP8A_OK;
}

int fp8a_dense_stats(uint64_t *out, int reset) {
    if (out == nullptr) return fail(FP8A_EINVAL, "null pointer");
    unsigned long long v[2] = {0, 0};
    if (hipDeviceSynchronize() != hipSuccess || hipMemcpyFromSymbol(v, HIP_SYMBOL(g_dense), sizeof(v)) != hipSuccess)
        return hip_check("fp8a_dense_stats");
    out[0] = v[0];
    out[1] = v[1];
    if (reset) {
        const unsigned long long z[2] = {0, 0};
        if (hipMemcpyToSymbol(HIP_SYMBOL(g_dense), z, sizeof(z)) != hipSuccess) return hip_check("fp8a_dense_stats");
    }
    return FP8A_OK;
}

int fp8a_decompose(const float *x, int64_t rows, int64_t cols, int64_t ld, int E, int M, const int32_t *bias,
                   int64_t bias_stride, uint32_t flags, int32_t *expo, int32_t *mant, fp8a_stream_t stream) {
    int rc = check_format(E, M);
    if (rc) return rc;
    if (rows < 0 || cols < 0 || ld < cols) return fail(FP8A_EINVAL, "bad decompose extents");
    const int64_t total = rows * cols;
    if (total == 0) return FP8A_OK;
    decompose_kernel<<<(unsigned)((total + 255) / 256), 256, 0, (hipStream_t)stream>>>(
        x, rows, cols, ld, E, M, bias, bias_stride, flags, expo, mant);
    return hip_check("fp8a_decompose");
}

int fp8a_quant(const float *x, int64_t n, int E, int M, const int32_t *bias, uint32_t flags, float *out,
               fp8a_stream_t stream) {
    int rc = check_format(E, M);
    if (rc) return rc;
    if (n <= 0) return FP8A_OK;
    quant_kernel<<<(unsigned)((n + 255) / 256), 256, 0, (hipStream_t)stream>>>(x, n, E, M, bias, flags, out);
    return hip_check("fp8a_quant");
}

static GemmArgs make_args(const float *A, int64_t lda, const float *B, int64_t sbk, int64_t sbn, float *C,
                          int64_t ldc, int64_t M, int64_t N, int64_t K, int E, int Mw, const int32_t *bA,
                          const int32_t *bB, int64_t bBs, const int32_t *bR, uint32_t flags) {
    GemmArgs a;
    memset(&a, 0, sizeof(a));
    a.A = A; a.lda = lda; a.B = B; a.sbk = sbk; a.sbn = sbn; a.C = C; a.ldc = ldc;
    a.M = M; a.N = N; a.K = K; a.E = E; a.Mw = Mw; a.kexp = 0x7F800000u; a.kdc = (uint32_t)(23 - Mw) << 23;
    a.bA = bA; a.bB = bB; a.bBs = bBs; a.bR = bR;
    a.flags = flags; a.nchw = 0; a.hw = 1; a.ctot = N; a.coff = 0;
    a.splits = 1; a.kchunk = K; a.part = nullptr;
    return a;
}

size_t fp8a_matmul_workspace_size(void) { return FLAG_BYTES; }

size_t fp8a_matmul_workspace_size_mnk(int64_t M, int64_t N, int64_t K) {
    if (M <= 0 || N <= 0 || K <= 0) return FLAG_BYTES;
    return gemm_workspace_bytes(M, N, K, 0);
}

int fp8a_matmul(const float *A, int64_t lda, const float *B, int64_t sbk, int64_t sbn, float *C, int64_t ldc,
                int64_t M, int64_t N, int64_t K, int E, int Mw, const int32_t *bA, const int32_t *bB,
                int64_t bB_stride, const int32_t *bR, const int32_t *table, uint32_t flags, void *workspace,
                size_t workspace_bytes, fp8a_stream_t stream) {
    if (lda < K || ldc < N) return fail(FP8A_EINVAL, "leading dimension smaller than extent");
    GemmArgs a = make_args(A, lda, B, sbk, sbn, C, ldc, M, N, K, E, Mw, bA, bB, bB_stride, bR, flags);
    return run_gemm(a, table, workspace, workspace_bytes, (hipStream_t)stream);
}

int fp8a_terms(const float *A, int64_t lda, const float *B, int64_t sbk, int64_t sbn, float *T, int64_t M,
               int64_t N, int64_t K, int E, int Mw, const int32_t *bA, const int32_t *bB, int64_t bB_stride,
               const int32_t *bR, const int32_t *table, uint32_t flags, fp8a_stream_t stream) {
    int rc = check_format(E, Mw);
    if (rc) return rc;
    GemmArgs a = make_args(A, lda, B, sbk, sbn, nullptr, 0, M, N, K, E, Mw, bA, bB, bB_stride, bR, flags);
    int mode;
    rc = pack_table(table, Mw, (flags & (F_APPROX | F_V5)) != 0, a.tab, mode);
    if (rc) return rc;
    const int64_t total = M * N * K;
    if (total == 0) return FP8A_OK;
    terms_kernel<<<(unsigned)((total + 255) / 256), 256, 0, (hipStream_t)stream>>>(a, T);
    return hip_check("fp8a_terms");
}

int fp8a_im2col(const float *x, float *out, int64_t Bn, int64_t Cin, int64_t H, int64_t W, int kh, int kw, int sh,
// ... 330 lines not shown
}

size_t fp8a_conv2d_qin_workspace_size(int64_t Bn, int64_t Cin, int64_t H, int64_t W, int64_t Cout, int kh, int kw,
                                      int sh, int sw, int ph, int pw, int dh, int dw, int groups) {
    const size_t n = fp8a_conv2d_workspace_size(Bn, Cin, H, W, Cout, kh, kw, sh, sw, ph, pw, dh, dw, groups);
    return n == 0 ? 0 : align256(n) + align256((size_t)(Bn * Cin * H * W) * sizeof(float));
}

int fp8a_conv2d_qin(const float *x, const float *w, float *y, int64_t Bn, int64_t Cin, int64_t H, int64_t W,
                    int64_t Cout, int kh, int kw, int sh, int sw, int ph, int pw, int dh, int dw, int groups, int E,
                    int Mw, const int32_t *bW, const int32_t *bR, const int32_t *table, uint32_t flags,
                    const float *bn, int act, float act_lo, float act_hi, const float *in_maxval, int in_nbits,
                    int in_mbits, int in_sign_bits, float *in_bias_out, int32_t *in_ibias_out, void *workspace,
                    size_t workspace_bytes, fp8a_stream_t stream) {
    if (!in_maxval || !in_bias_out || !in_ibias_out) return fail(FP8A_EINVAL, "null pointer");
    const int qE = in_nbits - in_sign_bits - in_mbits;
    if (in_mbits < 1 || qE < 1) return fail(FP8A_EFORMAT, "bad FP8 quantizer format");
    const size_t xq_bytes = align256((size_t)(Bn * Cin * H * W) * sizeof(float));
    if (workspace == nullptr || workspace_bytes < FLAG_BYTES + xq_bytes)
        return fail(FP8A_EINVAL, "conv2d_qin workspace too small");
    const size_t rest = (workspace_bytes - xq_bytes) & ~(size_t)255;
    float *xq = (float *)((char *)workspace + rest);
    return conv2d_impl(x, w, y, Bn, Cin, H, W, Cout, kh, kw, sh, sw, ph, pw, dh, dw, groups, E, Mw, nullptr, bW, bR,
                       table, flags, bn, act, act_lo, act_hi, workspace, rest, (hipStream_t)stream,
                       FqIn{in_maxval, qE, in_mbits, in_sign_bits}, in_bias_out, in_ibias_out, xq);
}


size_t fp8a_conv2d_block_workspace_size(int64_t Bn, int64_t Cin, int64_t H, int64_t W, int64_t Cout, int kh,
                                        int kw, int sh, int sw, int ph, int pw, int dh, int dw, int groups) {
    return fp8a_conv2d_qin_workspace_size(Bn, Cin, H, W, Cout, kh, kw, sh, sw, ph, pw, dh, dw, groups);
}

int fp8a_conv2d_block(const float *x, const float *w, float *y, int64_t Bn, int64_t Cin, int64_t H, int64_t W,
                      int64_t Cout, int kh, int kw, int sh, int sw, int ph, int pw, int dh, int dw, int groups, int E,
                      int Mw, const int32_t *bA, const int32_t *bW, const int32_t *bR, const int32_t *table,
                      uint32_t flags, const float *bn, int act, float act_lo, float act_hi, const float *in_maxval,
                      int in_nbits, int in_mbits, int in_sign_bits, float *in_bias_out, int32_t *in_ibias_out,
                      const float *res, int post_act, float post_lo, float post_hi, const float *out_maxval,
                      int out_nbits, int out_mbits, int out_sign_bits, float *out_bias_out, int32_t *out_ibias_out,
                      void *workspace, size_t workspace_bytes, fp8a_stream_t stream) {
    hipStream_t s = (hipStream_t)stream;
    if (post_act != 0 && post_act != 1) return fail(FP8A_EINVAL, "conv2d_block: post_act is 0 or 1");
    FqIn fin{}, fout{};
    if (in_maxval) {
        const int qE = in_nbits - in_sign_bits - in_mbits;
        if (in_mbits < 1 || qE < 1) return fail(FP8A_EFORMAT, "bad FP8 quantizer format");
        if (!in_bias_out || !in_ibias_out) return fail(FP8A_EINVAL, "null pointer");
        fin = FqIn{in_maxval, qE, in_mbits, in_sign_bits};
    } else if (!bA) {
        return fail(FP8A_EINVAL, "null pointer");
    }
    if (out_maxval) {
        const int qE = out_nbits - out_sign_bits - out_mbits;
        if (out_mbits < 1 || qE < 1) return fail(FP8A_EFORMAT, "bad FP8 quantizer format");
        if (!out_bias_out || !out_ibias_out) return fail(FP8A_EINVAL, "null pointer");
        fout = FqIn{out_maxval, qE, out_mbits, out_sign_bits};
    }
    const size_t xq_bytes = fin.mx ? align256((size_t)(Bn * Cin * H * W) * sizeof(float)) : 0;
    if (workspace == nullptr || workspace_bytes < FLAG_BYTES + xq_bytes)
        return fail(FP8A_EINVAL, "conv2d_block workspace too small");
    const size_t rest = (workspace_bytes - xq_bytes) & ~(size_t)255;
    float *xq = fin.mx ? (float *)((char *)workspace + rest) : nullptr;
    return conv2d_impl(x, w, y, Bn, Cin, H, W, Cout, kh, kw, sh, sw, ph, pw, dh, dw, groups, E, Mw,
                       fin.mx ? nullptr : bA, bW, bR, table, flags, bn, act, act_lo, act_hi, workspace, rest, s, fin,
                       in_bias_out, in_ibias_out, xq, res, post_act, post_lo, post_hi, fout, nullptr, EmitW{},
                       fout.mx ? out_bias_out : nullptr, fout.mx ? out_ibias_out : nullptr);
}

size_t fp8a_word_image_bytes(int64_t Bn, int64_t C, int64_t H, int64_t W, int ph, int pw) {
    if (Bn <= 0 || C <= 0 || H <= 0 || W <= 0 || ph < 0 || pw < 0) return 0;
    const WordImage wi = word_image(H, W, ph, pw);
    return FLAG_BYTES + align256((size_t)(Bn * C * wi.H * wi.W) * 4);
}

__global__ void emit_prep_kernel(uint32_t *hdr, FqIn fq, const int32_t *bR) {
    const float mx = *fq.mx, fb = fq_bias(mx, fq.E, fq.M);
    hdr[0] = 0u;
    hdr[1] = __float_as_uint(mx);
    hdr[2] = __float_as_uint(fb);
    hdr[3] = (uint32_t)(128 - (int)fb) << 23;
    hdr[4] = (uint32_t)*bR;
    hdr[5] = 0u;
}

__global__ void word_image_fill_kernel(uint32_t *img, int64_t words) {
    if (blockIdx.x == 0 && threadIdx.x < 64) img[threadIdx.x] = 0u;
    for (int64_t i = (int64_t)blockIdx.x * blockDim.x + threadIdx.x; i < words; i += (int64_t)gridDim.x * blockDim.x)
        img[64 + i] = XM_ZERO_WORD;
}

int fp8a_word_image_init(void *image, int64_t Bn, int64_t C, int64_t H, int64_t W, int ph, int pw,
                         fp8a_stream_t stream) {
    if (image == nullptr || fp8a_word_image_bytes(Bn, C, H, W, ph, pw) == 0) return fail(FP8A_EINVAL, "word image");
    if (((uintptr_t)image & 255) != 0) return fail(FP8A_EINVAL, "word image must be 256-byte aligned");
    const WordImage wi = word_image(H, W, ph, pw);
    const int64_t words = Bn * C * wi.H * wi.W;
    word_image_fill_kernel<<<(unsigned)std::min<int64_t>((words + 255) / 256, 8192), 256, 0, (hipStream_t)stream>>>(
        (uint32_t *)image, words);
    return hip_check("fp8a word image init");
}

int fp8a_conv2d_wants_image(int64_t Cout, int kh, int kw, int ph, int pw, int groups, int E, int Mw,
                            const int32_t *table, uint32_t flags, int sh, int sw, int dh, int dw) {
    if (Cout <= 1 || check_format(E, Mw) != FP8A_OK) return 0;
    TablePack tp;
    int mode;
    if (pack_table(table, Mw, (flags & F_APPROX) != 0, tp, mode) != FP8A_OK) return 0;
    if (groups > 1 && Cout == groups) {
        static const bool no_tbx = getenv("FP8A_NO_TBX") != nullptr;
        static const bool chain_tbx = getenv("FP8A_CHAIN_TBX") != nullptr && atoi(getenv("FP8A_CHAIN_TBX")) != 0;
        const bool tbx = chain_tbx && !no_tbx && ((E == 4 && Mw == 3) || (E == 5 && Mw == 2)) &&
                         (mode == TM_NONE || mode == TM_W1U) && (flags & F_S2N) && (flags & F_QBMA) &&
                         !(flags & (F_GCLIP | F_V5)) && kw == 3 && dw == 1 && sh == sw && (sw == 1 || sw == 2);
        (void)kh; (void)dh;
        return tbx ? 2 : 0;
    }
    if (groups != 1 || no_mx()) return 0;
    if (flags & F_V5) return (v5mx_form(Mw, flags, TM_V5) && ph == 0 && pw == 0) ? 3 : 0;
    if (!f8_form(E, Mw, flags & ~F_TB, mode)) return 0;
    if (kh == 1 && kw == 1 && ph == 0 && pw == 0) {
        const int64_t bnt = 16 * xm_ncg(Cout), ct = (Cout + bnt - 1) / bnt;
        if (ct <= af32_maxct(sh, sw)) return 0;
    }
    return 1;
}

int fp8a_conv2d_chain(const float *x, const float *w, float *y, int64_t Bn, int64_t Cin, int64_t H, int64_t W,
                      int64_t Cout, int kh, int kw, int sh, int sw, int ph, int pw, int dh, int dw, int groups, int E,
                      int Mw, const int32_t *bA, const int32_t *bW, const int32_t *bR, const int32_t *table,
                      uint32_t flags, const float *bn, int act, float act_lo, float act_hi, const float *in_maxval,
                      int in_nbits, int in_mbits, int in_sign_bits, float *in_bias_out, int32_t *in_ibias_out,
                      const float *res, int post_act, float post_lo, float post_hi, const float *out_maxval,
                      int out_nbits, int out_mbits, int out_sign_bits, float *out_bias_out, int32_t *out_ibias_out,
                      void *in_image, void *out_image, int next_ph, int next_pw, const float *next_maxval,
                      int next_nbits, int next_mbits, int next_sign_bits, const int32_t *next_bR, int next_Mw,
                      int next_form, void *workspace, size_t workspace_bytes, fp8a_stream_t stream) {
    if (post_act != 0 && post_act != 1) return fail(FP8A_EINVAL, "conv2d_chain: post_act is 0 or 1");
    hipStream_t s = (hipStream_t)stream;
    if ((in_image && ((uintptr_t)in_image & 255)) || (out_image && ((uintptr_t)out_image & 255)))
        return fail(FP8A_EINVAL, "word images must be 256-byte aligned");
    FqIn fin{}, fout{};
    if (in_maxval) {
        const int qE = in_nbits - in_sign_bits - in_mbits;
        if (in_mbits < 1 || qE < 1) return fail(FP8A_EFORMAT, "bad FP8 quantizer format");
        if (!in_bias_out || !in_ibias_out) return fail(FP8A_EINVAL, "null pointer");
        fin = FqIn{in_maxval, qE, in_mbits, in_sign_bits};
    } else if (!bA) {
        return fail(FP8A_EINVAL, "null pointer");
    }
    if (out_maxval) {
        const int qE = out_nbits - out_sign_bits - out_mbits;
        if (out_mbits < 1 || qE < 1) return fail(FP8A_EFORMAT, "bad FP8 quantizer format");
        if (!out_bias_out || !out_ibias_out) return fail(FP8A_EINVAL, "null pointer");
        fout = FqIn{out_maxval, qE, out_mbits, out_sign_bits};
    }
    EmitW em{};
    if (out_image) {
        const int64_t Ho = (H + 2 * ph - dh * (kh - 1) - 1) / sh + 1, Wo = (W + 2 * pw - dw * (kw - 1) - 1) / sw + 1;
        const int qE = next_nbits - next_sign_bits - next_mbits;
        if (!next_maxval || !next_bR || next_mbits < 1 || qE < 1 || !(next_Mw == 2 || next_Mw == 3) || next_ph < 0 ||
            next_pw < 0)
            return fail(FP8A_EINVAL, "bad next-convolution parameters for the word image");
        if (next_form < 0 || next_form > 2) return fail(FP8A_EINVAL, "bad word image form");
        const WordImage wi = next_form == 1 ? word_image(Ho, Wo, 0, 0) : word_image(Ho, Wo, next_ph, next_pw);
        const bool dwp = groups > 1 && Cin == groups && Cout == groups;
// ... 261 lines not shown
```

### fp8_quantization_amd/csrc/fp8approx_common.h

```cpp
#pragma once
#include <hip/hip_runtime.h>
#include <stdint.h>
#include <string.h>

#include <algorithm>
#include <atomic>
#include <cmath>
#include <cstdlib>
#include <cstdio>
#include <string>

#include "../../include/fp8approx.h"
#include "fp8approx_device.h"

namespace fp8a {

enum TMode : int { TM_NONE = 0, TM_W1U = 1, TM_W2S1 = 2, TM_W2U1 = 3, TM_W2S2 = 4, TM_W2U2 = 5, TM_LUT = 6,
                   TM_QAMAA = 7 ,
                   TM_V5 = 8 ,
                   TM_F8 = 9  };

struct TablePack {
    uint32_t rows[64][2];
    int8_t raw[1024];
};

struct FqIn {
    const float *mx;
    int E, M, S;
};

__device__ __forceinline__ float fq_bias(float mx, int E, int M) {
    return rintf((float)(1 << E) - log2f(mx) + log2f(2.0f - p2(-M)) - 1.0f);
}

__device__ __forceinline__ float fq_step(float xc, int k) {
    const float t = (k >= -126) ? xc * p2(-k) : (xc * 18446744073709551616.0f) * p2(-k - 64);
    const float r = rintf(t) * p2(k);
    return k < -149 ? rintf(xc * __builtin_huge_valf()) * p2(k) : r;
}
__device__ __forceinline__ float fq_apply_lit(float xc, float bias, int M) {
    int e;
    frexpf(xc, &e);
    const float ls = (xc == 0.0f) ? 1.0f : fmaxf((float)(e - 1) + bias, 1.0f);
    return fq_step(xc, (int)(ls - (float)M - bias));
}
__device__ __forceinline__ float fq_apply(float v, float mx, float bias, int M, int sign_bits) {
    return fq_apply_lit(fminf(fmaxf(v, sign_bits ? -mx : 0.0f), mx), bias, M);
}

struct EmitW {
    uint32_t *w;
    uint32_t *invalid;
    int awH, awW, awph, awpw;
    int Wo;
    uint32_t hw_mul, hw_shift, wo_mul, wo_shift;
    uint32_t hw;
    FqIn fq;
    const int32_t *bR;
    int Mw;
    int form;
};

struct GemmArgs {
    const float *A;
    int64_t lda;
    const float *B;
    int64_t sbk, sbn;
    float *C;
    int64_t ldc;
    int64_t M, N, K;
    int E, Mw;
    uint32_t kexp, kdc;
    const int32_t *bA;
    const int32_t *bB;
    int64_t bBs;
    const int32_t *bR;
    uint32_t flags;
    int nchw;
    int64_t hw, ctot, coff;
    uint32_t *flag;
    uint8_t *urow, *ucol, *utile;
    int64_t nur, nuc;
    int splits;
    int64_t kchunk;
    float *part;
    int conv;
    const float *X;
    int64_t Cin, H, W, Ho, Wo, cbase;
    int kh, kw, sh, sw, ph, pw, dh, dw;
    uint32_t kk_mul, kk_shift, kw_mul, kw_shift;
    const float *qmax;
    int qE, qM, qsign;
    const float2 *ep;
    int ep_act;
    float ep_lo, ep_hi;
    const uint32_t *aw;
    int64_t awld, aw_c;
    int64_t awH, awW;
    int awph, awpw;
    int wfmt;
    int ttf7;
    int af32;
    int xncg;
    const uint2 *bqw;
    const uint32_t *lutw;
    const uint16_t *ebr;
    int xm_vmin;
    int64_t npad;
    FqIn fqin;
    float *fq_bias;
    int32_t *fq_ibias;
    const float *res;
    int post_act;
    float post_lo, post_hi;
    FqIn post_fq;
    EmitW em;
    const uint32_t *gate;
    const uint32_t *in_img;
    TablePack tab;
    uint32_t *flag_out;
    uint4 *arena_clr;
    uint32_t arena_clr16;
    float *post_bout;
    int32_t *post_ibout;
};

constexpr uint32_t FB_ANY = 1u, FB_ALL = 32u;
constexpr uint32_t FB_HALF = 64u;
constexpr uint8_t UT_EXACT = 1u, UT_HALF = 2u;

__device__ __forceinline__ uint32_t fb_bits(const GemmArgs &p, bool all = false) {
    return (all || p.urow == nullptr) ? (FB_ANY | FB_ALL) : FB_ANY;
}

__device__ __forceinline__ void arena_clear(uint4 *clr, uint32_t n16) {
    for (uint32_t i = blockIdx.x * blockDim.x + threadIdx.x; i < n16; i += gridDim.x * blockDim.x)
        clr[i] = make_uint4(0u, 0u, 0u, 0u);
}

__device__ __forceinline__ void fb_rows(const GemmArgs &p, int64_t m_lo, int64_t m_hi) {
    if (p.urow == nullptr || m_hi <= m_lo) return;
    for (int64_t u = m_lo >> 6; u <= (m_hi - 1) >> 6; ++u) p.urow[u] = 1;
}
__device__ __forceinline__ void fb_col(const GemmArgs &p, int64_t n) {
    if (p.ucol != nullptr) p.ucol[n >> 6] = 1;
}
__device__ __forceinline__ void fb_tile(const GemmArgs &p, int64_t m0, int64_t rows, int64_t n0,
                                        uint8_t mark = UT_EXACT) {
    if (p.utile == nullptr) return;
    const int64_t hi = min(m0 + rows, p.M);
    for (int64_t u = m0 >> 6; u <= (hi - 1) >> 6; ++u) p.utile[u * p.nuc + (n0 >> 6)] = mark;
}

__device__ __forceinline__ float post_bias(const GemmArgs &p) {
    return p.post_fq.mx ? fq_bias(*p.post_fq.mx, p.post_fq.E, p.post_fq.M) : 0.0f;
}

__device__ __forceinline__ float gelu_erf(float x) {
    return x * 0.5f * (1.0f + erff(x * (float)M_SQRT1_2));
}

template <bool GELU = true>
__device__ __forceinline__ float post_tail(const GemmArgs &p, float v, float pb) {
    if (p.post_act == 1) v = fminf(fmaxf(v, p.post_lo), p.post_hi);
    else if (GELU && p.post_act == 2) v = gelu_erf(v);
    if (p.post_fq.mx) v = fq_apply(v, *p.post_fq.mx, pb, p.post_fq.M, p.post_fq.S);
    return v;
}

template <bool GELU = true>
__device__ __forceinline__ float post1(const GemmArgs &p, int64_t o, float v, float pb) {
    if (p.res) v += p.res[o];
    return post_tail<GELU>(p, v, pb);
}

template <bool GELU = true>
__device__ __forceinline__ float4 post4(const GemmArgs &p, int64_t o, float4 v, float pb) {
    if (p.res) {
        const float4 r = *reinterpret_cast<const float4 *>(p.res + o);
        v.x += r.x; v.y += r.y; v.z += r.z; v.w += r.w;
    }
    return make_float4(post_tail<GELU>(p, v.x, pb), post_tail<GELU>(p, v.y, pb), post_tail<GELU>(p, v.z, pb), post_tail<GELU>(p, v.w, pb));
}

__device__ __forceinline__ float epi(const float2 *ep, int act, float lo, float hi, int64_t c, float x) {
    if (ep == nullptr) return x;
    const float2 e = ep[c];
    const float v = __fmaf_rn(x, e.x, e.y);
    return act ? fminf(fmaxf(v, lo), hi) : v;
}

static inline void fastdiv_params(uint32_t d, uint32_t &mul, uint32_t &shift) {
    uint32_t l = 0;
    while ((1ull << l) < d) ++l;
    shift = l;
    mul = (uint32_t)(((1ull << 32) * ((1ull << l) - d)) / d + 1);
}

__device__ __forceinline__ uint32_t fastdiv(uint32_t n, uint32_t mul, uint32_t shift) {
    return (__umulhi(n, mul) + n) >> shift;
}

constexpr int BM = 64, BN = 64, BK = 16, TM = 4, TN = 4, NT = 256;
constexpr int AP = BM + 4, BP = BN + 4;

__device__ __forceinline__ uint32_t xm_word_a(float x, int M, int xb, uint32_t emnA, int bR, bool &ok);
__host__ __device__ constexpr int xm_xbias(int Mw);

constexpr uint32_t XM_ZERO_WORD = 253u << 23;

struct EmitCtx {
    float mx, fb;
    uint32_t emn;
    int bR;
};
__device__ __forceinline__ EmitCtx emit_ctx(const GemmArgs &p) {
    EmitCtx e{};
    if (p.em.w == nullptr) return e;
    const uint4 h = *reinterpret_cast<const uint4 *>(p.em.invalid);
    e.mx = __uint_as_float(__builtin_amdgcn_readfirstlane(h.y));
    e.fb = __uint_as_float(__builtin_amdgcn_readfirstlane(h.z));
    e.emn = __builtin_amdgcn_readfirstlane(h.w);
    e.bR = __builtin_amdgcn_readfirstlane((int)p.em.invalid[4]);
    return e;
}
__device__ __forceinline__ uint32_t emit_word(const GemmArgs &p, const EmitCtx &e, float v, bool &ok) {
    const float q = fq_apply(v, e.mx, e.fb, p.em.fq.M, p.em.fq.S);
    if (p.em.form) {
        const uint32_t u = __float_as_uint(q), ua = u & 0x7FFFFFFFu, M = (uint32_t)p.em.Mw;
        ok = ok && (ua == 0u || ((ua & ((1u << (23 - M)) - 1u)) == 0u && ua >= 0x20800000u && ua <= 0x58800000u));
        return ua == 0u ? 0u : ((u & 0xFF800000u) | (((ua >> (23 - M)) & ((1u << M) - 1u)) << 3));
    }
    return xm_word_a(q, p.em.Mw, xm_xbias(p.em.Mw), e.emn, e.bR, ok);
}
__device__ __forceinline__ uint32_t emit_index(const GemmArgs &p, uint32_t uo, uint32_t &wo) {
    const uint32_t plane = fastdiv(uo, p.em.hw_mul, p.em.hw_shift), pix = uo - plane * p.em.hw;
    const uint32_t ho = fastdiv(pix, p.em.wo_mul, p.em.wo_shift);
    wo = pix - ho * (uint32_t)p.em.Wo;
    return (plane * (uint32_t)p.em.awH + ho + (uint32_t)p.em.awph) * (uint32_t)p.em.awW + wo + (uint32_t)p.em.awpw;
}
__device__ __forceinline__ void wave_max_atomic(uint32_t *dst, uint32_t v) {
#pragma unroll
    for (int off = 32; off >= 1; off >>= 1) v = max(v, (uint32_t)__shfl_xor((int)v, off));
    if ((threadIdx.x & 63) == 0 && v != 0u && v > __hip_atomic_load(dst, __ATOMIC_RELAXED, __HIP_MEMORY_SCOPE_AGENT))
        atomicMax(dst, v);
}
__device__ __forceinline__ uint32_t word_sehi(uint32_t w) { return w == XM_ZERO_WORD ? 0u : 255u - (w >> 23); }

__device__ __forceinline__ void emit1(const GemmArgs &p, const EmitCtx &e, int64_t o, float v, uint32_t &sehi) {
    uint32_t wo;
    const uint32_t wi = emit_index(p, (uint32_t)o, wo);
    bool ok = true;
    const uint32_t w = emit_word(p, e, v, ok);
    p.em.w[wi] = w;
    sehi = max(sehi, word_sehi(w));
    if (!ok) atomicOr(p.em.invalid, 1u);
}
__device__ __forceinline__ void emit4(const GemmArgs &p, const EmitCtx &e, int64_t o, float4 v, uint32_t &sehi) {
    uint32_t wo;
    const uint32_t wi = emit_index(p, (uint32_t)o, wo);
    bool ok0 = true, ok1 = true, ok2 = true, ok3 = true;
    const uint4 w = make_uint4(emit_word(p, e, v.x, ok0), emit_word(p, e, v.y, ok1), emit_word(p, e, v.z, ok2),
                               emit_word(p, e, v.w, ok3));
    sehi = max(max(sehi, max(word_sehi(w.x), word_sehi(w.y))), max(word_sehi(w.z), word_sehi(w.w)));
    if (wo + 3 < (uint32_t)p.em.Wo && (wi & 3u) == 0u) {
        *reinterpret_cast<uint4 *>(p.em.w + wi) = w;
    } else {
        p.em.w[wi] = w.x;
        uint32_t wo1;
        p.em.w[emit_index(p, (uint32_t)o + 1, wo1)] = w.y;
        p.em.w[emit_index(p, (uint32_t)o + 2, wo1)] = w.z;
        p.em.w[emit_index(p, (uint32_t)o + 3, wo1)] = w.w;
    }
    if (!(ok0 && ok1 && ok2 && ok3)) atomicOr(p.em.invalid, 1u);
}

__device__ __forceinline__ int64_t out_index(const GemmArgs &p, int64_t m, int64_t n) {
    if (!p.nchw) return m * p.ldc + n;
    const int64_t img = m / p.hw, pix = m - img * p.hw;
    return (img * p.ctot + p.coff + n) * p.hw + pix;
}

__device__ __forceinline__ bool stage_decode(float x, int M, uint32_t emn, bool s2n, float &c, uint32_t &m) {
    const uint32_t u = __float_as_uint(x);
    const uint32_t ua = u & 0x7FFFFFFFu;
    const uint32_t ex = ua & 0x7F800000u;
    const bool sub = ua < emn;
    const uint32_t sh = (uint32_t)(23 - M) + (sub ? ((emn - ex) >> 23) : 0u);
    const bool grid = (sh < 24u) ? ((ua & ((1u << sh) - 1u)) == 0u) : (ua == 0u);
    const bool win = (ua == 0u) || (ua >= 0x20800000u  && ua <= 0x58800000u );
    m = (ua >> (23 - M)) & ((1u << M) - 1u);
    c = (ua == 0u || (!s2n && sub)) ? 0.0f : __uint_as_float(u & 0xFF800000u);
    return grid && win;
}

template <bool EMIT = true, bool GELU = true>
__device__ __forceinline__ void store_tile(const GemmArgs &p, int64_t split, int64_t m0, int64_t n0, int ty, int tx,
                                           float (&acc)[TM][TN]) {
    const bool partial = p.splits > 1;
    float *const C = partial ? p.part + split * p.M * p.N : p.C;
    const int64_t ldc = partial ? p.N : p.ldc, ctot = partial ? p.N : p.ctot, coff = partial ? 0 : p.coff;
    const int64_t nb = n0 + tx * TN;
    if (!partial && p.ep != nullptr) {
#pragma unroll
        for (int j = 0; j < TN; ++j) {
            const int64_t ch = p.coff + min<int64_t>(nb + j, p.N - 1);
#pragma unroll
            for (int i = 0; i < TM; ++i) acc[i][j] = epi(p.ep, p.ep_act, p.ep_lo, p.ep_hi, ch, acc[i][j]);
        }
    }
    const float pb = partial ? 0.0f : post_bias(p);
    const GemmArgs &q = p;
    const bool emit = EMIT && !partial && p.em.w != nullptr;
    const EmitCtx ec = EMIT ? emit_ctx(p) : EmitCtx{};
    uint32_t sehi = 0;
    auto fin1 = [&](int64_t o, float v) {
        if (partial) return v;
        v = post1<GELU>(q, o, v, pb);
        if (emit) emit1(q, ec, o, v, sehi);
        return v;
    };
    auto fin4 = [&](int64_t o, float4 v) {
        if (partial) return v;
        v = post4<GELU>(q, o, v, pb);
        if (emit) emit4(q, ec, o, v, sehi);
        return v;
    };
    if (!p.nchw) {
#pragma unroll
        for (int i = 0; i < TM; ++i) {
            const int64_t m = m0 + ty * TM + i;
            if (m >= p.M) continue;
            if (nb + TN <= p.N && ((ldc & 3) == 0) && ((((uintptr_t)C) & 15) == 0)) {
                *reinterpret_cast<float4 *>(&C[m * ldc + nb]) =
                    fin4(m * ldc + nb, make_float4(acc[i][0], acc[i][1], acc[i][2], acc[i][3]));
            } else {
#pragma unroll
                for (int j = 0; j < TN; ++j)
                    if (nb + j < p.N) C[m * ldc + nb + j] = fin1(m * ldc + nb + j, acc[i][j]);
            }
        }
    } else {
        const int64_t mb = m0 + ty * TM;
        const int64_t img = mb / p.hw, pix = mb - img * p.hw;
        const bool vec = (pix + TM <= p.hw) && (mb + TM <= p.M) && ((p.hw & 3) == 0) &&
                         ((((uintptr_t)C) & 15) == 0);
        if (vec) {
#pragma unroll
            for (int j = 0; j < TN; ++j)
                if (nb + j < p.N) {
                    const int64_t o = (img * ctot + coff + nb + j) * p.hw + pix;
                    *reinterpret_cast<float4 *>(&C[o]) = fin4(o, make_float4(acc[0][j], acc[1][j], acc[2][j], acc[3][j]));
                }
        } else {
#pragma unroll
            for (int i = 0; i < TM; ++i) {
                const int64_t m = mb + i;
                if (m >= p.M) continue;
                const int64_t im = m / p.hw, px = m - im * p.hw;
#pragma unroll
                for (int j = 0; j < TN; ++j)
                    if (nb + j < p.N) {
                        const int64_t o = (im * ctot + coff + nb + j) * p.hw + px;
                        C[o] = fin1(o, acc[i][j]);
                    }
            }
        }
    }
    if (emit) wave_max_atomic(p.em.invalid + 5, sehi);
}

}
```

### fp8_quantization_amd/csrc/fp8approx_launch.h

```cpp
#pragma once
#include "fp8approx_common.h"

namespace fp8a {

void launch_fast_p0(int mode, bool gclip, const GemmArgs &a, dim3 grid, hipStream_t s);
void launch_fast_p1(int mode, bool gclip, const GemmArgs &a, dim3 grid, hipStream_t s);
void launch_fast_p2(int mode, bool gclip, const GemmArgs &a, dim3 grid, hipStream_t s);
void launch_fast_p3(int mode, bool gclip, const GemmArgs &a, dim3 grid, hipStream_t s);

void launch_f8mx_xf0(const GemmArgs &a, hipStream_t s);
void launch_f8mx_xf1(const GemmArgs &a, hipStream_t s);
void launch_f8mx_xf2(const GemmArgs &a, hipStream_t s);
int f8mx_clock_xf0(unsigned long long *v, bool reset);
int f8mx_clock_xf1(unsigned long long *v, bool reset);
int f8mx_clock_xf2(unsigned long long *v, bool reset);

void launch_tt(const GemmArgs &a, dim3 grid, hipStream_t s);
int tt_rerun_stats(unsigned long long *v, bool reset);

void launch_v5mx(const GemmArgs &a, hipStream_t s);

}
```

### fp8_quantization_amd/csrc/gemm_f8mx.h

```cpp
#pragma once
#include "fp8approx_common.h"

namespace fp8a {

typedef int xm_v8i __attribute__((ext_vector_type(8)));
typedef float xm_v16f __attribute__((ext_vector_type(16)));
typedef float xm_v4f __attribute__((ext_vector_type(4)));
typedef short xm_s2 __attribute__((ext_vector_type(2)));
typedef unsigned short xm_u2 __attribute__((ext_vector_type(2)));
typedef __bf16 xm_b2 __attribute__((ext_vector_type(2)));

constexpr int XM_NPAIR = 81;
constexpr int XM_LUT_WORDS = XM_NPAIR * 8;
constexpr uint32_t XM_ROW_SHIFT = 3, XM_ROW_MASK = 0x78u;
constexpr int XBK = 8;
constexpr int XM_TTK = 16 * 32 + 16;
constexpr int XM_CP = BN + 1;

template <int XF>
struct XmFmt {
    static constexpr int M = XF ? 2 : 3;
    static constexpr int XB = XF ? 15 : 7;
};
__device__ __forceinline__ bool xm_needs_halving(const GemmArgs &p, bool af32, int bA, int bR) {
// ... 48 lines not shown
    static_assert(BMT % 64 == 0 && BMT % SR == 0, "tile rows");
    static_assert((TTK % 64) >= 16 && (TTK % 64) <= 48, "odd K-steps of the table build must not share banks");
};

__device__ __forceinline__ bool xm_bias_ok(int b) { return b >= -100 && b <= 120; }

__device__ __forceinline__ uint32_t xm_lut_word(const TablePack &tab, int e, int M) {
    const int pr = e >> 3, ma = e & 7, n = 1 << M;
    const float ulp = M == 3 ? 0.125f : 0.25f;
    const float bound = M == 3 ? 1.8671875f : 1.6875f;
    uint32_t w = 0;
    if (ma >= n) return 0u;
#pragma unroll
    for (int h = 0; h < 2; ++h) {
        const int cd = h ? (pr / 9) : (pr % 9);
        if (cd >= n) continue;
        const float t = (float)tab.raw[ma * n + cd];
        float v = __fmaf_rn(1.0f + ulp * ma, 1.0f + ulp * cd, -t * ulp);
        v = fminf(v, __uint_as_float(__float_as_uint(v) & 0x7F800000u) * bound);
        w |= (__float_as_uint(v) >> 16) << (16 * h);
    }
    return w;
}

__device__ __forceinline__ uint32_t xm_word_a(float x, int M, int xb, uint32_t emnA, int bR, bool &ok) {
    float c;
    uint32_t mc;
    ok = stage_decode(x, M, emnA, true, c, mc);
    const uint32_t cb = __float_as_uint(c);
    const int se = 254 + xb - bR - (int)((cb >> 23) & 0xFFu);
    if ((cb & 0x7FFFFFFFu) == 0u) return XM_ZERO_WORD;
    ok = ok && se >= 1 && se <= 252;
    return ((uint32_t)min(max(se, 1), 252) << 23) | (((cb >> 31) * 8u + mc) << XM_ROW_SHIFT);
}

constexpr int TT_RS = 68;
constexpr uint32_t TT_EXP = 0xFF800000u;
__device__ __forceinline__ uint32_t tt_word_a(float x, int M, uint32_t emnA, bool &ok) {
    float c;
    uint32_t mc;
    ok = stage_decode(x, M, emnA, true, c, mc);
    const uint32_t cb = __float_as_uint(c);
    if ((cb & 0x7FFFFFFFu) == 0u) return 0u;
    return (cb & TT_EXP) | (mc * (uint32_t)(4 * TT_RS));
}

constexpr int TT16_XK = 4;
constexpr int TT16_RS = 34;
constexpr int TT16_KS = 16 * TT16_RS;
constexpr uint32_t TT16_RSH = 2 * TT16_RS;
constexpr uint32_t TT16_EXP2 = 0xFC00FC00u;
constexpr int TT16_IMG = 2048;

typedef _Float16 tt16_h2 __attribute__((ext_vector_type(2)));
typedef _Float16 tt16_h8 __attribute__((ext_vector_type(8)));
typedef float tt16_f4 __attribute__((ext_vector_type(4)));


__device__ __forceinline__ uint32_t tt16_pow2(int e, uint32_t sign) { return sign | ((uint32_t)(e + 15) << 10); }

__device__ __forceinline__ uint32_t tt16_word_a(float x, uint32_t emnA, int bA, bool &ok, bool &win) {
    float c;
    uint32_t mc;
    ok = stage_decode(x, 4, emnA, true, c, mc);
    const uint32_t cb = __float_as_uint(c);
    if ((cb & 0x7FFFFFFFu) == 0u) return 0u;
    const int e = (int)((cb >> 23) & 0xFFu) - 127 + bA - 1;
    ok = ok && e >= -14 && e <= 15;
    win = win && e <= 7;
    const uint32_t h = tt16_pow2(min(max(e, -14), 15), (cb >> 16) & 0x8000u);
    return (h << 16) | h | (mc * TT16_RSH);
}

__device__ __forceinline__ uint32_t v5_word_a(float v, const DFmt &f) {
    int e, m;
    exact_dec(v, f, true, e, m);
    const uint32_t h = (v < 0.0f ? 0x8000u : 0u) | ((uint32_t)(e * (1 << f.M) + m) << 5);
    return h * 0x10001u;
}

__device__ __forceinline__ void xm_record_se(const GemmArgs &p, uint32_t sehi) {
    if (p.Mw == 2 && p.wfmt == 0) wave_max_atomic(p.flag + 1, sehi);
}

#if FP8A_OWN_F8MX_DECODE
__global__ __launch_bounds__(256) void xm_decode_a(const GemmArgs p) {
    const float fmx = p.fqin.mx ? *p.fqin.mx : 0.0f;
    const float fbias = p.fqin.mx ? fq_bias(fmx, p.fqin.E, p.fqin.M) : 0.0f;
    const int bA = p.fqin.mx ? (int)fbias : *p.bA, bR = *p.bR;
    if (p.fqin.mx && blockIdx.x == 0 && blockIdx.y == 0 && threadIdx.x == 0) {
        *p.fq_bias = fbias;
        *p.fq_ibias = bA;
    }
    if (p.gate != nullptr && __hip_atomic_load(p.gate, __ATOMIC_RELAXED, __HIP_MEMORY_SCOPE_AGENT) == 0u) {
        if (p.Mw == 2 && p.wfmt == 0 && blockIdx.x == 0 && blockIdx.y == 0 && threadIdx.x == 0)
            atomicMax(p.flag + 1, p.gate[5]);
        return;
    }
    const uint32_t emnA = (uint32_t)(128 - bA) << 23;
    const bool biasbad = !(xm_bias_ok(bA) && xm_bias_ok(bR));
    bool bad = biasbad, win = true;
    const int64_t orows = p.conv ? p.Ho * p.Wo : 1;
    uint32_t *const out = const_cast<uint32_t *>(p.aw);
    const int64_t hw = p.H * p.W;
    const int64_t rows = p.conv ? p.M / (p.Ho * p.Wo) : p.M, cols = p.conv ? p.aw_c * p.awH * p.awW : p.awld;
    uint32_t sehi = 0;
    const DFmt fv5 = dfmt(p.E, p.Mw, bA, false);
    auto word = [&](float v, bool &ok) {
        if (p.fqin.mx) v = fq_apply(v, fmx, fbias, p.fqin.M, p.fqin.S);
        if (p.wfmt == 4) return v5_word_a(v, fv5);
        if (p.wfmt == 2) return tt16_word_a(v, emnA, bA, ok, win);
        if (p.wfmt) return tt_word_a(v, p.Mw, emnA, ok);
        const uint32_t w = xm_word_a(v, p.Mw, xm_xbias(p.Mw), emnA, bR, ok);
        sehi = max(sehi, word_sehi(w));
        return w;
    };
    const uint32_t zw = p.wfmt ? 0u : XM_ZERO_WORD;
    auto st1 = [&](int64_t i, uint32_t w) { out[i] = w; };
    auto st4 = [&](int64_t i, uint4 w) { *reinterpret_cast<uint4 *>(out + i) = w; };
    if (p.conv && (p.awph | p.awpw)) {
        const uint32_t uW = (uint32_t)p.W, uH = (uint32_t)p.H, Wp = (uint32_t)p.awW, Hp = (uint32_t)p.awH;
        const uint32_t hwin = uH * uW, ph = (uint32_t)p.awph, pw = (uint32_t)p.awpw, pr = Wp - uW - pw;
        const uint32_t nin = (uint32_t)p.aw_c * hwin;
        const bool v4 = (uW % 4 == 0) && (Wp % 4 == 0) && (pw % 4 == 0) &&
                        (((uintptr_t)(p.X + p.cbase * hw) & 15) == 0) && ((p.Cin * hw) % 4 == 0) &&
                        (((uintptr_t)out & 15) == 0) && (cols % 4 == 0);
        const uint32_t per = v4 ? 4u : 1u, nb = 2 * ph * Wp + (pw + pr) * uH;
        const uint32_t tstride = gridDim.x * blockDim.x, t0 = blockIdx.x * blockDim.x + threadIdx.x;
        for (int64_t r = blockIdx.y; r < rows; r += gridDim.y) {
            const float *in = p.X + (r * p.Cin + p.cbase) * hw;
            const int64_t o = r * cols;
            bool badr = false;
            for (uint32_t e = per * t0; e < nin; e += per * tstride) {
                const uint32_t c = e / hwin, t = e - c * hwin, hy = t / uW, wx = t - hy * uW;
                const int64_t d = o + (c * Hp + hy + ph) * Wp + pw + wx;
                if (v4) {
                    const float4 v = *reinterpret_cast<const float4 *>(in + e);
                    bool ok0 = true, ok1 = true, ok2 = true, ok3 = true;
                    st4(d, make_uint4(word(v.x, ok0), word(v.y, ok1), word(v.z, ok2), word(v.w, ok3)));
                    badr |= !(ok0 && ok1 && ok2 && ok3);
                } else {
                    bool ok = true;
                    st1(d, word(in[e], ok));
                    badr |= !ok;
                }
            }
            if (badr) fb_rows(p, r * orows, (r + 1) * orows);
            bad |= badr;
            for (uint32_t j = t0; j < (uint32_t)p.aw_c * nb; j += tstride) {
                const uint32_t c = j / nb, t = j - c * nb;
                uint32_t row, col;
                if (t < 2 * ph * Wp) {
                    const uint32_t rr = t / Wp;
                    row = rr < ph ? rr : uH + rr;
                    col = t - rr * Wp;
                } else {
                    const uint32_t u = t - 2 * ph * Wp, rr = u / (pw + pr), sc = u - rr * (pw + pr);
                    row = ph + rr;
                    col = sc < pw ? sc : uW + sc;
                }
                st1(o + (c * Hp + row) * Wp + col, zw);
            }
        }
        if (__syncthreads_or(bad ? 1 : 0) && threadIdx.x == 0) atomicOr(p.flag, fb_bits(p, biasbad));
        if (__syncthreads_or(win ? 0 : 1) && threadIdx.x == 0) atomicOr(p.flag, 4u);
        xm_record_se(p, sehi);
        return;
    }
    const int64_t lim0 = p.conv ? cols : p.K, istride = p.conv ? p.Cin * hw : p.lda;
    const float *in0 = p.conv ? p.X + p.cbase * hw : p.A;
    const bool vec = (lim0 % 4 == 0) && (cols % 4 == 0) && (istride % 4 == 0) && (((uintptr_t)in0 & 15) == 0) &&
                     (((uintptr_t)out & 15) == 0);
    if (vec) {
        const uint32_t c4n = (uint32_t)(cols / 4), lim4 = (uint32_t)(lim0 / 4), nq = (uint32_t)rows * c4n;
        const uint32_t nthr = gridDim.x * gridDim.y * blockDim.x;
        const uint32_t tid = (blockIdx.y * gridDim.x + blockIdx.x) * blockDim.x + threadIdx.x;
        constexpr int XU = 4;
        const uint32_t dr = nthr / c4n, dc = nthr - dr * c4n;
        uint32_t r = tid / c4n, c = tid - r * c4n;
        for (uint32_t q = tid; q < nq; q += XU * nthr) {
            float4 v[XU];
            uint32_t rr[XU], cc[XU];
#pragma unroll
            for (int u = 0; u < XU; ++u) {
                rr[u] = r;
                cc[u] = c;
                if (q + u * nthr < nq && c < lim4)
                    v[u] = *reinterpret_cast<const float4 *>(in0 + (int64_t)r * istride + 4 * c);
                c += dc;
                r += dr;
                if (c >= c4n) {
                    c -= c4n;
                    ++r;
                }
            }
#pragma unroll
            for (int u = 0; u < XU; ++u) {
                if (q + u * nthr >= nq) break;
                uint4 w = make_uint4(zw, zw, zw, zw);
                if (cc[u] < lim4) {
                    bool ok0 = true, ok1 = true, ok2 = true, ok3 = true;
                    w = make_uint4(word(v[u].x, ok0), word(v[u].y, ok1), word(v[u].z, ok2), word(v[u].w, ok3));
                    if (!(ok0 && ok1 && ok2 && ok3)) {
                        fb_rows(p, (int64_t)rr[u] * orows, ((int64_t)rr[u] + 1) * orows);
                        bad = true;
                    }
                }
                st4((int64_t)rr[u] * cols + 4 * cc[u], w);
            }
        }
    } else {
        for (int64_t r = blockIdx.y; r < rows; r += gridDim.y) {
            const float *in = p.conv ? p.X + (r * p.Cin + p.cbase) * hw : p.A + r * p.lda;
            const int64_t lim = p.conv ? cols : p.K;
            const int64_t o = r * cols;
            bool badr = false;
            for (int64_t i = (int64_t)blockIdx.x * blockDim.x + threadIdx.x; i < cols;
                 i += (int64_t)gridDim.x * blockDim.x) {
                bool ok = true;
                st1(o + i, (i < lim) ? word(in[i], ok) : zw);
                badr |= !ok;
            }
            if (badr) fb_rows(p, r * orows, (r + 1) * orows);
            bad |= badr;
        }
    }
    if (__syncthreads_or(bad ? 1 : 0) && threadIdx.x == 0) atomicOr(p.flag, fb_bits(p, biasbad));
    if (__syncthreads_or(win ? 0 : 1) && threadIdx.x == 0) atomicOr(p.flag, 4u);
    xm_record_se(p, sehi);
}
#else
__global__ void xm_decode_a(const GemmArgs p);
#endif

#if FP8A_OWN_F8MX_DECODE
__global__ __launch_bounds__(256) void xm_decode_b(const GemmArgs p, int64_t kpad) {
    const int bA = p.af32 ? 0 : *p.bA, bR = *p.bR;
    const bool biasbad = !(xm_bias_ok(bA) && xm_bias_ok(bR));
    bool bad = biasbad;
    const int64_t hq = p.npad / 2, n = kpad * hq;
    uint2 *const bq = const_cast<uint2 *>(p.bqw);
    if (blockIdx.x == 0)
        for (int e = threadIdx.x; e < XM_LUT_WORDS; e += blockDim.x) const_cast<uint32_t *>(p.lutw)[e] = xm_lut_word(p.tab, e, p.Mw);
    const int64_t stride = (int64_t)gridDim.x * blockDim.x;
    for (int64_t i = (int64_t)blockIdx.x * blockDim.x + threadIdx.x; i < n; i += stride) {
        const int64_t k = i / hq, q = i - k * hq;
        float c[2];
        uint32_t mc[2];
#pragma unroll
        for (int h = 0; h < 2; ++h) {
            const int64_t col = 2 * q + h;
            c[h] = 0.0f;
            mc[h] = 0;
            if (k < p.K && col < p.N) {
                const int bb = p.bB[col * p.bBs];
                const bool ok = stage_decode(p.B[k * p.sbk + col * p.sbn], p.Mw, (uint32_t)(128 - bb) << 23, true,
                                             c[h], mc[h]) && xm_bias_ok(bb);
                if (!ok) fb_col(p, col);
                bad |= !ok;
            }
        }
        uint32_t add = 0, code[2];
#pragma unroll
        for (int h = 0; h < 2; ++h) {
            const uint32_t cb = __float_as_uint(c[h]);
            if ((cb & 0x7FFFFFFFu) == 0u) {
                code[h] = 8u;
            } else {
                code[h] = mc[h];
                const uint32_t eb = ((cb >> 23) & 0xFFu) - 127u;
                add |= ((((cb >> 31) << 15) + (eb << 7)) & 0xFFFFu) << (16 * h);
            }
        }
        bq[i] = make_uint2(add, (code[0] + 9u * code[1]) * 32u);
    }
    if (p.Mw == 2 && p.ebr != nullptr) {
        const int64_t ng = p.npad / 16;
        uint32_t bmax = 0;
        for (int64_t i = (int64_t)blockIdx.x * blockDim.x + threadIdx.x; i < kpad * ng; i += stride) {
            const int64_t k = i / ng, g = i - k * ng;
            int emax = -128, emin = 127;
            for (int j = 0; j < 16 && k < p.K; ++j) {
                const int64_t col = 16 * g + j;
                if (col >= p.N) break;
                float c;
                uint32_t mc;
                stage_decode(p.B[k * p.sbk + col * p.sbn], p.Mw, (uint32_t)(128 - p.bB[col * p.bBs]) << 23, true, c, mc);
                const uint32_t cb = __float_as_uint(c);
                if ((cb & 0x7FFFFFFFu) == 0u) continue;
                const int e = (int)((cb >> 23) & 0xFFu) - 127;
                emax = max(emax, e);
                emin = min(emin, e);
            }
            const_cast<uint16_t *>(p.ebr)[i] = (uint16_t)((emax + 128) | ((emin + 128) << 8));
            bmax = max(bmax, (uint32_t)(emax + 128));
        }
        wave_max_atomic(p.flag + 2, bmax);
    }
    if (__syncthreads_or(bad ? 1 : 0) && threadIdx.x == 0) atomicOr(p.flag, fb_bits(p, biasbad));
}
#else
__global__ void xm_decode_b(const GemmArgs p, int64_t kpad);
#endif

#if FP8A_OWN_F8MX
#ifndef FP8A_CLOCK_STAMP
#define FP8A_CLOCK_STAMP 0
#endif
__device__ unsigned long long g_clk[3];
#if FP8A_CLOCK_STAMP
#define FP8A_CLK_BEGIN const uint64_t clk_t0 = __builtin_amdgcn_s_memtime(), clk_r0 = __builtin_amdgcn_s_memrealtime();
#define FP8A_CLK_END                                                                                   \
    if (threadIdx.x == 0) {                                                                            \
        const uint64_t clk_t1 = __builtin_amdgcn_s_memtime(), clk_r1 = __builtin_amdgcn_s_memrealtime(); \
        atomicAdd(&g_clk[0], (unsigned long long)(clk_t1 - clk_t0));                                   \
        atomicAdd(&g_clk[1], (unsigned long long)(clk_r1 - clk_r0));                                   \
        atomicAdd(&g_clk[2], 1ull);                                                                    \
    }
#else
#define FP8A_CLK_BEGIN
#define FP8A_CLK_END
#endif
#ifndef XM_WAVES
#define XM_WAVES 5
#endif
#ifndef XM_WAVES_PLAIN
#define XM_WAVES_PLAIN (XM_BDMA ? 6 : XM_WAVES)
#endif
template <bool AF32, bool EMIT> struct XmWaves { static constexpr int value = XM_WAVES; };
template <> struct XmWaves<false, false> { static constexpr int value = XM_WAVES_PLAIN; };
template <int NCG, int RB, bool AF32, int XF, bool EMIT>
__global__ __launch_bounds__(256, (XmWaves<AF32, EMIT>::value)) void gemm_f8mx_kernel(const GemmArgs p) {
    using Cf = XmCfg<NCG, RB>;
    constexpr int XM = XmFmt<XF>::M, XB = XmFmt<XF>::XB;
    constexpr int NT = Cf::NT, BMT = Cf::BMT, BNT = Cf::BNT, TTK = Cf::TTK, APR = Cf::APR;
    constexpr int BU = Cf::BU, NBU = Cf::NBU, TXN = Cf::TXN, SR = Cf::SR, CP = Cf::CP;
    __shared__ __attribute__((aligned(16))) typename Cf::Smem smu;
    auto &sm = smu.st;
    FP8A_CLK_BEGIN

    const int tid = threadIdx.x, lane = tid & 63, wv = tid >> 6;
    const int wvu = __builtin_amdgcn_readfirstlane(wv);
    const int wc = wvu % NCG, wr = wvu / NCG;
    const int64_t num_mt = (p.M + BMT - 1) / BMT;
    const int64_t tiles = num_mt * ((p.N + BNT - 1) / BNT);
    const int64_t bid = (int64_t)blockIdx.x % tiles, split = (int64_t)blockIdx.x / tiles;
    const int64_t m0 = (bid % num_mt) * BMT;
    const int64_t n0 = (bid / num_mt) * BNT;
    if (XF == 2 && !xm_half_gate(p, m0, BMT, n0, BNT)) return;
    const int kbeg = (int)(split * p.kchunk), kend = (int)min(p.K, (int64_t)kbeg + p.kchunk), K32 = (int)p.K;
    const int bR = *p.bR;
    float fmx = 0.0f, fbias = 0.0f;
    int bA = 0;
    bool abad = false, biasbad = false;
    if (AF32) {
        fmx = p.fqin.mx ? *p.fqin.mx : 0.0f;
        fbias = p.fqin.mx ? fq_bias(fmx, p.fqin.E, p.fqin.M) : 0.0f;
        bA = p.fqin.mx ? (int)fbias : *p.bA;
        if (p.fqin.mx && blockIdx.x == 0 && tid == 0) {
            *p.fq_bias = fbias;
            *p.fq_ibias = bA;
        }
        biasbad = !(xm_bias_ok(bA) && xm_bias_ok(bR));
    }
    const uint32_t emnA = (uint32_t)(128 - bA) << 23;

    for (int e = 4 * tid; e < XM_LUT_WORDS; e += 4 * NT)
        *reinterpret_cast<uint4 *>(&sm.lut[e]) = *reinterpret_cast<const uint4 *>(&p.lutw[e]);

    const uint32_t hq8 = (uint32_t)(p.npad / 2) * 8u;
    const int q4 = tid & 3, btx = (tid >> 3) % TXN;
    constexpr int BKU = 2 * (NT / (8 * TXN));
    const int bkk0 = 2 * (tid / (8 * TXN)) + ((tid >> 2) & 1);
    const uint32_t boff0 = (uint32_t)(kbeg + bkk0) * hq8 + (uint32_t)(n0 / 2 + 2 * btx) * 8u;
    const bool build = NBU % NT == 0 || tid < NBU;
#if XM_BDMA
    const float *bsrc = reinterpret_cast<const float *>(p.bqw) +
                        ((size_t)(kbeg + tid / TXN) * (hq8 / 4) + (size_t)(n0 / 2 + 2 * (tid % TXN)) * 2);
    (void)boff0;
#else
    const __amdgpu_buffer_rsrc_t brsrc =
        __builtin_amdgcn_make_buffer_rsrc(const_cast<uint2 *>(p.bqw), (short)0, -1, 0x00020000);
#endif

    const int arow = p.conv ? lane : (tid >> 2), akp = p.conv ? wvu : (tid & 3);
    uint32_t aoff[APR];
    const uint32_t phw = AF32 ? (uint32_t)(p.H * p.W) : (uint32_t)(p.awH * p.awW), uW = (uint32_t)p.awW;
#pragma unroll
    for (int i = 0; i < APR; ++i) {
        const int64_t m = min(m0 + arow + 64 * i, p.M - 1);
        if (p.conv) {
            const int64_t hw = p.Ho * p.Wo, img = m / hw, pix = m - img * hw, ho = pix / p.Wo, wo = pix - ho * p.Wo;
            if (AF32)
                aoff[i] = (uint32_t)(4 * ((img * p.Cin + p.cbase) * (int64_t)phw + ho * p.sh * p.W + wo * p.sw));
            else
                aoff[i] = (uint32_t)(4 * (img * p.aw_c * (int64_t)phw + ho * p.sh * p.awW + wo * p.sw + (p.awpw - p.pw)));
        } else {
            aoff[i] = (uint32_t)(4 * (m * (AF32 ? p.lda : p.awld) + 2 * akp));
        }
    }
    const __amdgpu_buffer_rsrc_t arsrc =
        AF32 ? __builtin_amdgcn_make_buffer_rsrc(const_cast<float *>(p.conv ? p.X : p.A), (short)0, -1, 0x00020000)
             : __builtin_amdgcn_make_buffer_rsrc(const_cast<uint32_t *>(p.aw), (short)0, -1, 0x00020000);
    const int khw = p.kh * p.kw;
    uint32_t wa[APR][2];
#if !XM_BDMA
    uint4 wbq[BU];
#endif
    auto load_tile = [&](int k0) {
#pragma unroll
        for (int r = 0; r < 2; ++r) {
            if (AF32 && !p.conv) {
                const uint32_t k = (uint32_t)min(k0 + 2 * akp + r, K32 - 1);
#pragma unroll
                for (int i = 0; i < APR; ++i)
                    wa[i][r] = __builtin_amdgcn_raw_buffer_load_b32(arsrc, (int)(aoff[i] - 8u * (uint32_t)akp + 4u * k), 0, 0);
                continue;
            }
            uint32_t ko;
            if (AF32) {
                ko = 4u * (uint32_t)min(k0 + 2 * akp + r, K32 - 1) * phw;
            } else if (p.conv) {
                const int k = min(k0 + 2 * akp + r, K32 - 1);
                const uint32_t c = fastdiv((uint32_t)k, p.kk_mul, p.kk_shift);
                const uint32_t t = (uint32_t)k - c * (uint32_t)khw;
                const uint32_t ky = fastdiv(t, p.kw_mul, p.kw_shift);
                const uint32_t kx = t - ky * (uint32_t)p.kw;
                ko = 4u * (c * phw + ky * (uint32_t)p.dh * uW + kx * (uint32_t)p.dw);
            } else {
                ko = 4u * (uint32_t)(k0 + r);
            }
            ko = __builtin_amdgcn_readfirstlane(ko);
#pragma unroll
            for (int i = 0; i < APR; ++i) {
                wa[i][r] = __builtin_amdgcn_raw_buffer_load_b32(arsrc, (int)aoff[i], (int)ko, 0);
            }
        }
#if XM_BDMA
        if (tid < XBK * TXN)
            __builtin_amdgcn_global_load_lds(bsrc + (size_t)(k0 - kbeg) * (hq8 / 4), reinterpret_cast<float *>(&sm.bw[64 * wvu]), 16, 0, 0);
#else
        if (build) {
            const uint32_t kb = __builtin_amdgcn_readfirstlane((uint32_t)(k0 - kbeg) * hq8);
#pragma unroll
            for (int u = 0; u < BU; ++u)
                wbq[u] = __builtin_bit_cast(uint4, __builtin_amdgcn_raw_buffer_load_b128(
                                                       brsrc, (int)boff0, (int)(kb + (uint32_t)(u * BKU) * hq8), 0));
        }
#endif
    };
    load_tile(kbeg);

    xm_v8i sel;
    {
        const int n = lane & 15;
#pragma unroll
        for (int v = 0; v < 8; ++v) {
            uint32_t w = 0;
#pragma unroll
            for (int b = 0; b < 4; ++b)
                if (((4 * v + b) & 15) == n) w |= 0x38u << (8 * b);
            sel[v] = (int)w;
        }
    }
    xm_v4f dq[RB];
#pragma unroll
    for (int b = 0; b < RB; ++b) dq[b] = (xm_v4f){0.0f, 0.0f, 0.0f, 0.0f};
    xm_v8i av = {0, 0, 0, 0, 0, 0, 0, 0};
    const char *lut = reinterpret_cast<const char *>(sm.lut);
    const uint32_t wvo = (uint32_t)wc * 512u;
    typedef const volatile __attribute__((address_space(3))) uint64_t xm_lds_u64;
#if XM_BDMA
    __builtin_amdgcn_s_waitcnt(0x0F70);
#endif
    __syncthreads();

    for (int k0 = kbeg; k0 < kend; k0 += XBK) {
        if (AF32) {
#pragma unroll
            for (int i = 0; i < APR; ++i)
#pragma unroll
                for (int r = 0; r < 2; ++r) {
                    if (k0 + 2 * akp + r >= K32) {
                        wa[i][r] = XM_ZERO_WORD;
                    } else {
                        float v = __uint_as_float(wa[i][r]);
                        if (p.fqin.mx) v = fq_apply(v, fmx, fbias, p.fqin.M, p.fqin.S);
                        bool ok = true;
                        wa[i][r] = xm_word_a(v, XM, XB, emnA, bR, ok);
                        if (!ok) {
                            const int64_t m = min(m0 + arow + 64 * i, p.M - 1);
                            fb_rows(p, m, m + 1);
                            abad = true;
                        }
                    }
                }
        }
        if (!AF32 && p.conv) {
#pragma unroll
            for (int r = 0; r < 2; ++r)
                if (k0 + 2 * akp + r >= K32)
#pragma unroll
                    for (int i = 0; i < APR; ++i) wa[i][r] = XM_ZERO_WORD;
        }
#pragma unroll
        for (int i = 0; i < APR; ++i)
            *reinterpret_cast<uint2 *>(&sm.aw[akp][2 * (arow + 64 * i)]) = make_uint2(wa[i][0], wa[i][1]);
        if (build) {
#pragma unroll
            for (int u = 0; u < BU; ++u) {
#if XM_BDMA
                const uint4 b = sm.bw[(bkk0 + u * BKU) * TXN + btx];
#else
                const uint4 b = wbq[u];
#endif
                const uint2 s0 = *reinterpret_cast<const uint2 *>(lut + b.y + 8 * q4);
                const uint2 s1 = *reinterpret_cast<const uint2 *>(lut + b.w + 8 * q4);
                const xm_u2 a0 = __builtin_bit_cast(xm_u2, b.x), a1 = __builtin_bit_cast(xm_u2, b.z);
                const xm_u2 n0 = __builtin_bit_cast(xm_u2, b.x ^ 0x80008000u), n1 = __builtin_bit_cast(xm_u2, b.z ^ 0x80008000u);
                auto pk = [](uint32_t v, xm_u2 ad) { return __builtin_bit_cast(uint32_t, __builtin_bit_cast(xm_u2, v) + ad); };
                uint32_t *d = &sm.tt[bkk0 + u * BKU][btx * 32 + q4 * 4];
                *reinterpret_cast<uint4 *>(d) = make_uint4(pk(s0.x, a0), pk(s1.x, a1), pk(s0.y, a0), pk(s1.y, a1));
                *reinterpret_cast<uint4 *>(d + 16) = make_uint4(pk(s0.x, n0), pk(s1.x, n1), pk(s0.y, n0), pk(s1.y, n1));
            }
        }
        __syncthreads();
        if (k0 + XBK < kend) load_tile(k0 + XBK);

        {
            const int r16 = lane & 15, g = lane >> 4;
            const uint32_t base = wvo + (uint32_t)(2 * g) * (uint32_t)(TTK * 4);
            const char *tt0 = reinterpret_cast<const char *>(&sm.tt[0][0]);
            uint32_t thr = 0u;
            if (XF == 2) {
                const int64_t ng = p.npad / 16, e0 = (int64_t)(k0 + 2 * g) * ng + (n0 / 16 + wc);
                const uint32_t r0 = p.ebr[e0], r1 = p.ebr[e0 + ng];
                const uint32_t thi0 = (uint32_t)max(112 + (int)(r0 & 0xFFu) - 128, 0);
                const uint32_t thi1 = (uint32_t)max(112 + (int)(r1 & 0xFFu) - 128, 0);
                const uint32_t tok0 = (uint32_t)min(max(140 + (int)(r0 >> 8) - 128 + p.xm_vmin, 0), 252);
                const uint32_t tok1 = (uint32_t)min(max(140 + (int)(r1 >> 8) - 128 + p.xm_vmin, 0), 252);
                thr = thi0 | (thi1 << 8) | (tok0 << 16) | (tok1 << 24);
            }
#pragma unroll
            for (int b = 0; b < RB; ++b) {
                const uint2 aw2 = *reinterpret_cast<const uint2 *>(&sm.aw[g][2 * (16 * (RB * wr + b) + r16)]);
                uint32_t awh[2] = {aw2.x, aw2.y};
                int sca = 127;
                if (XF == 2) {
                    const uint32_t se0 = awh[0] >> 23, se1 = awh[1] >> 23;
                    const uint32_t n0b = (se0 - (thr & 0xFFu) - 1u) >> 31, n1b = (se1 - ((thr >> 8) & 0xFFu) - 1u) >> 31;
                    const uint32_t o0b = ((se0 - ((thr >> 16) & 0xFFu) - 1u) >> 31) | ((252u - se0) >> 31);
                    const uint32_t o1b = ((se1 - (thr >> 24) - 1u) >> 31) | ((252u - se1) >> 31);
                    const uint32_t bits = n0b | (n1b << 1) | (o0b << 2) | (o1b << 3);
                    const auto sw16 = __builtin_amdgcn_permlane16_swap(bits, bits, false, false);
                    const uint32_t pb = (g & 1) ? sw16[0] : sw16[1];
                    const uint32_t halve = (bits | pb) & ((bits & pb) >> 2) & 3u;
                    awh[0] += (halve & 1u) << 23;
                    awh[1] += (halve >> 1) << 23;
                    const auto sw32 = __builtin_amdgcn_permlane32_swap(halve, halve, false, false);
                    const uint32_t ph = (g >= 2) ? sw32[0] : sw32[1];
                    sca = 127 + (int)(((g == 1 || g == 2) ? ph : halve) >> (g >> 1) & 1u);
                }
#pragma unroll
                for (int h = 0; h < 2; ++h) {
                    uint32_t a;
                    asm("v_and_or_b32 %0, %1, %2, %3" : "=v"(a) : "v"(awh[h]), "s"(XM_ROW_MASK), "v"(base));
                    __builtin_assume((a & 7u) == 0u);
                    xm_lds_u64 *ttk = (xm_lds_u64 *)(tt0 + h * TTK * 4);
                    uint2 v[4];
#pragma unroll
                    for (int c = 0; c < 4; ++c) {
                        const uint64_t w = ttk[(a >> 3) + 16 * c];
                        v[c] = make_uint2((uint32_t)w, (uint32_t)(w >> 32));
                    }
                    const float sc = __uint_as_float(awh[h]);
#pragma unroll
                    for (int c = 0; c < 4; ++c) {
                        xm_s2 cv;
                        if (XF) {
                            asm("v_cvt_scalef32_pk_bf8_bf16 %0, %1, %2" : "=v"(cv) : "v"(v[c].x), "v"(sc));
                            cv = __builtin_amdgcn_cvt_scalef32_pk_bf8_bf16(cv, __builtin_bit_cast(xm_b2, v[c].y), sc, true);
                        } else {
                            asm("v_cvt_scalef32_pk_fp8_bf16 %0, %1, %2" : "=v"(cv) : "v"(v[c].x), "v"(sc));
                            cv = __builtin_amdgcn_cvt_scalef32_pk_fp8_bf16(cv, __builtin_bit_cast(xm_b2, v[c].y), sc, true);
                        }
                        av[4 * h + c] = __builtin_bit_cast(int, cv);
                    }
                }
                dq[b] = __builtin_amdgcn_mfma_scale_f32_16x16x128_f8f6f4(av, sel, dq[b], XF ? 1 : 0, 0, 0, sca, 0, 127);
            }
        }
#if XM_BDMA
        __builtin_amdgcn_s_waitcnt(0x0F70);
#endif
        __syncthreads();
    }

    bool nan = false;
#pragma unroll
    for (int b = 0; b < RB; ++b)
#pragma unroll
        for (int i = 0; i < 4; ++i) nan |= !__builtin_isfinite(dq[b][i]);
    const bool tnan = __syncthreads_or(nan ? 1 : 0) != 0;
    const bool tbad = AF32 && __syncthreads_or((abad || biasbad) ? 1 : 0) != 0;
    if ((tnan || tbad) && tid == 0) {
        if (XF == 1 && tnan && xm_needs_halving(p, AF32, AF32 ? bA : 0, bR)) {
// ... 38 lines not shown
```

### fp8_quantization_amd/csrc/k_f8mx.hip

```cpp
#ifndef FP8A_XF_PART
#error "k_f8mx.hip is compiled once per part: -DFP8A_XF_PART=0..2"
#endif
#define FP8A_OWN_F8MX 1
#define FP8A_OWN_F8MX_DECODE (FP8A_XF_PART == 0)
#include "fp8approx_launch.h"
#include "gemm_f8mx.h"

namespace fp8a {

template <int NCG, int RB, int XF>
static void launch_shape(const GemmArgs &a, hipStream_t s) {
    using Cf = XmCfg<NCG, RB>;
    const int64_t xt = ((a.M + Cf::BMT - 1) / Cf::BMT) * ((a.N + Cf::BNT - 1) / Cf::BNT);
    const dim3 g((unsigned)(xt * a.splits));
    const bool emit = a.em.w != nullptr && a.splits == 1;
    if (a.af32) {
        if (emit) gemm_f8mx_kernel<NCG, RB, true, XF, true><<<g, Cf::NT, 0, s>>>(a);
        else gemm_f8mx_kernel<NCG, RB, true, XF, false><<<g, Cf::NT, 0, s>>>(a);
    } else {
        if (emit) gemm_f8mx_kernel<NCG, RB, false, XF, true><<<g, Cf::NT, 0, s>>>(a);
        else gemm_f8mx_kernel<NCG, RB, false, XF, false><<<g, Cf::NT, 0, s>>>(a);
    }
}

template <int XF>
static void launch_xf(const GemmArgs &a, hipStream_t s) {
    if (a.xncg == 1) {
        launch_shape<1, 4, XF>(a, s);
    } else if constexpr (XF == 2) {
        launch_shape<2, 4, XF>(a, s);
    } else {
        if (a.xncg == 2) launch_shape<2, 4, XF>(a, s);
        else launch_shape<4, 8, XF>(a, s);
    }
}

static int clock_read(unsigned long long *v, bool reset) {
    if (hipMemcpyFromSymbol(v, HIP_SYMBOL(g_clk), 3 * sizeof(unsigned long long)) != hipSuccess) return -1;
    if (reset) {
        const unsigned long long z[3] = {0, 0, 0};
        if (hipMemcpyToSymbol(HIP_SYMBOL(g_clk), z, sizeof(z)) != hipSuccess) return -1;
    }
    return 0;
}

#if FP8A_XF_PART == 0
void launch_f8mx_xf0(const GemmArgs &a, hipStream_t s) { launch_xf<0>(a, s); }
int f8mx_clock_xf0(unsigned long long *v, bool reset) { return clock_read(v, reset); }
#elif FP8A_XF_PART == 1
void launch_f8mx_xf1(const GemmArgs &a, hipStream_t s) { launch_xf<1>(a, s); }
int f8mx_clock_xf1(unsigned long long *v, bool reset) { return clock_read(v, reset); }
#else
void launch_f8mx_xf2(const GemmArgs &a, hipStream_t s) { launch_xf<2>(a, s); }
int f8mx_clock_xf2(unsigned long long *v, bool reset) { return clock_read(v, reset); }
#endif

}
```

### include/fp8approx.h

```cpp
#ifndef FP8APPROX_H
#define FP8APPROX_H

#include <stdint.h>
#include <stddef.h>

#ifdef __cplusplus
extern "C" {
#endif

#define FP8A_APPROX 1u
#define FP8A_S2N    2u
#define FP8A_QBMA   4u
#define FP8A_GCLIP  8u
#define FP8A_TB     16u
#define FP8A_V5     32u
#define FP8A_OFUF   64u
#define FP8A_OF_OPT 128u
#define FP8A_UF_OPT 256u

#define FP8A_OK       0
#define FP8A_EINVAL  -1
#define FP8A_EFORMAT -2
#define FP8A_EHIP    -3

typedef void *fp8a_stream_t;

const char *fp8a_version(void);
const char *fp8a_last_error(void);

int fp8a_fallback_stats(uint64_t *out, int reset);

int fp8a_path_stats(uint64_t *out, int reset);

size_t fp8a_flag_arena_slot_bytes(fp8a_stream_t stream);

int fp8a_kernel_timing(int enable);
int fp8a_kernel_time(double *out, int reset);

int fp8a_set_option(const char *name, int value);

#define FP8A_DENSE_E4M3 0
#define FP8A_DENSE_E5M2 1
#define FP8A_DENSE_BF16 2
size_t fp8a_dense_matmul_workspace_size(int64_t M, int64_t N, int64_t K);
int fp8a_dense_matmul(const float *A, int64_t sam, int64_t sak, const float *B, int64_t sbk, int64_t sbn, float *C,
                      int64_t ldc, int64_t M, int64_t N, int64_t K, int fmt, void *workspace, size_t workspace_bytes,
                      fp8a_stream_t stream);
size_t fp8a_dense_conv2d_workspace_size(int64_t Bn, int64_t Cin, int64_t H, int64_t W, int64_t Cout, int kh, int kw,
                                        int sh, int sw, int ph, int pw, int dh, int dw);
int fp8a_dense_conv2d(const float *x, const float *w, float *y, int64_t Bn, int64_t Cin, int64_t H, int64_t W,
                      int64_t Cout, int kh, int kw, int sh, int sw, int ph, int pw, int dh, int dw, int fmt,
                      void *workspace, size_t workspace_bytes, fp8a_stream_t stream);
int fp8a_grouped_conv2d(const float *x, const float *w, float *y, int64_t Bn, int64_t Cin, int64_t H, int64_t W,
                        int64_t Cout, int groups, int kh, int kw, int sh, int sw, int ph, int pw, int dh, int dw,
                        fp8a_stream_t stream);
int fp8a_dense_conv2d_fused(const float *x, const float *w, float *y, int64_t Bn, int64_t Cin, int64_t H, int64_t W,
                            int64_t Cout, int kh, int kw, int sh, int sw, int ph, int pw, int dh, int dw, int groups,
                            int fmt, const float *w_maxval, int w_per_channel, int w_nbits, int w_mbits,
                            int w_sign_bits, float *w_bias_out, int32_t *w_ibias_out, const float *in_maxval,
                            int in_nbits, int in_mbits, int in_sign_bits, float *in_bias_out, int32_t *in_ibias_out,
                            const float *res_maxval, int res_nbits, int res_mbits, int res_sign_bits,
                            float *res_bias_out, int32_t *res_ibias_out, const float *bn, int act, float act_lo,
                            float act_hi, const float *out_maxval, int out_nbits, int out_mbits, int out_sign_bits,
                            float *out_bias_out, int32_t *out_ibias_out, void *workspace, size_t workspace_bytes,
                            fp8a_stream_t stream);
int fp8a_dense_stats(uint64_t *out, int reset);

int fp8a_clock_stats(uint64_t *out, int reset);

int fp8a_decompose(const float *x, int64_t rows, int64_t cols, int64_t ld, int E, int M,
                   const int32_t *bias, int64_t bias_stride, uint32_t flags,
                   int32_t *expo, int32_t *mant, fp8a_stream_t stream);

int fp8a_quant(const float *x, int64_t n, int E, int M, const int32_t *bias, uint32_t flags,
               float *out, fp8a_stream_t stream);

size_t fp8a_matmul_workspace_size(void);
size_t fp8a_matmul_workspace_size_mnk(int64_t M, int64_t N, int64_t K);
int fp8a_matmul(const float *A, int64_t lda, const float *B, int64_t sbk, int64_t sbn,
                float *C, int64_t ldc, int64_t M, int64_t N, int64_t K, int E, int Mw,
                const int32_t *bA, const int32_t *bB, int64_t bB_stride, const int32_t *bR,
                const int32_t *table, uint32_t flags, void *workspace, size_t workspace_bytes,
                fp8a_stream_t stream);

int fp8a_terms(const float *A, int64_t lda, const float *B, int64_t sbk, int64_t sbn, float *T,
               int64_t M, int64_t N, int64_t K, int E, int Mw, const int32_t *bA,
               const int32_t *bB, int64_t bB_stride, const int32_t *bR, const int32_t *table,
               uint32_t flags, fp8a_stream_t stream);

size_t fp8a_conv2d_workspace_size(int64_t Bn, int64_t Cin, int64_t H, int64_t W, int64_t Cout,
                                  int kh, int kw, int sh, int sw, int ph, int pw, int dh, int dw,
                                  int groups);
int fp8a_conv2d(const float *x, const float *w, float *y, int64_t Bn, int64_t Cin, int64_t H,
                int64_t W, int64_t Cout, int kh, int kw, int sh, int sw, int ph, int pw, int dh,
                int dw, int groups, int E, int Mw, const int32_t *bA, const int32_t *bW,
                const int32_t *bR, const int32_t *table, uint32_t flags, void *workspace,
                size_t workspace_bytes, fp8a_stream_t stream);

int fp8a_conv2d_bn_act(const float *x, const float *w, float *y, int64_t Bn, int64_t Cin,
                       int64_t H, int64_t W, int64_t Cout, int kh, int kw, int sh, int sw, int ph,
                       int pw, int dh, int dw, int groups, int E, int Mw, const int32_t *bA,
                       const int32_t *bW, const int32_t *bR, const int32_t *table, uint32_t flags,
                       const float *bn, int act, float act_lo, float act_hi, void *workspace,
                       size_t workspace_bytes, fp8a_stream_t stream);

size_t fp8a_conv2d_qin_workspace_size(int64_t Bn, int64_t Cin, int64_t H, int64_t W, int64_t Cout,
                                      int kh, int kw, int sh, int sw, int ph, int pw, int dh, int dw,
                                      int groups);
int fp8a_conv2d_qin(const float *x, const float *w, float *y, int64_t Bn, int64_t Cin, int64_t H,
                    int64_t W, int64_t Cout, int kh, int kw, int sh, int sw, int ph, int pw, int dh,
                    int dw, int groups, int E, int Mw, const int32_t *bW, const int32_t *bR,
                    const int32_t *table, uint32_t flags, const float *bn, int act, float act_lo,
                    float act_hi, const float *in_maxval, int in_nbits, int in_mbits,
                    int in_sign_bits, float *in_bias_out, int32_t *in_ibias_out, void *workspace,
                    size_t workspace_bytes, fp8a_stream_t stream);
// ... 73 lines not shown
```

Measured before the change: 12650 images/s.

## Skip negated-sign table build in f8mx GEMM when no negative activation words exist

The A-decode and epilogue paths now OR together the emitted activation words and record, into flag slots, whether any of them carries the sign bit. The f8mx GEMM reads these flags per block, and when no negative A word was seen it builds only the positive half of the per-K lookup table in shared memory, skipping the negated half. This is meant to cut LDS writes and ALU work in the table-build step for post-ReLU inputs, which are all non-negative. It adds atomics and flag reads across stages, plus some debug counters, and its correctness depends on the sign flags being complete.

Measured after the change: 13090 images/s (median of 6 runs). 3.5% higher.

```diff
diff --git a/fp8_quantization_amd/_lib.py b/fp8_quantization_amd/_lib.py
--- a/fp8_quantization_amd/_lib.py
+++ b/fp8_quantization_amd/_lib.py
@@ -18,6 +18,7 @@
            "fp8a_fp8_quantize", "fp8a_matmul_qamaa", "fp8a_conv2d_qamaa", "fp8a_matmul_block_workspace_size",
            "fp8a_matmul_block", "fp8a_dense_matmul_workspace_size", "fp8a_dense_matmul",
            "fp8a_dense_conv2d_workspace_size", "fp8a_dense_conv2d", "fp8a_grouped_conv2d", "fp8a_dense_conv2d_fused", "fp8a_dense_stats", "fp8a_clock_stats",
+           "fp8a_xm_sign_stats", "fp8a_splitk_stats",
            "fp8a_word_image_bytes", "fp8a_word_image_init", "fp8a_conv2d_chain", "fp8a_conv2d_wants_image",
            "fp8a_flag_arena_slot_bytes")
 
@@ -89,6 +90,8 @@
                                      P, I, I, I, P, P, P, SZ, P], I),
         "fp8a_dense_stats": ([P, I], I),
         "fp8a_clock_stats": ([P, I], I),
+        "fp8a_xm_sign_stats": ([P, I], I),
+        "fp8a_splitk_stats": ([P, I], I),
         "fp8a_flag_arena_slot_bytes": ([P], SZ),
     }
     for name, (args, res) in sig.items():
@@ -187,6 +190,20 @@
     return dict(fp32_launches=int(out[0]), fp32_units=int(out[1]))
 
 
+def xm_sign_stats(reset=False):
+    L = load()
+    out = (ctypes.c_uint64 * 2)()
+    check(L.fp8a_xm_sign_stats(ctypes.cast(out, ctypes.c_void_p), 1 if reset else 0), "fp8a_xm_sign_stats")
+    return dict(half=int(out[0]), full=int(out[1]))
+
+
+def splitk_stats(reset=False):
+    L = load()
+    out = (ctypes.c_uint64 * 1)()
+    check(L.fp8a_splitk_stats(ctypes.cast(out, ctypes.c_void_p), 1 if reset else 0), "fp8a_splitk_stats")
+    return int(out[0])
+
+
 def clock_stats(reset=False):
     L = load()
     out = (ctypes.c_uint64 * 3)()
diff --git a/fp8_quantization_amd/csrc/conv_tbx.h b/fp8_quantization_amd/csrc/conv_tbx.h
--- a/fp8_quantization_amd/csrc/conv_tbx.h
+++ b/fp8_quantization_amd/csrc/conv_tbx.h
@@ -335,7 +335,7 @@
     const char *lut = reinterpret_cast<const char *>(sL);
     const int nqd = (p.Wo + 3) >> 2, pq = p.RB * nqd;
     float emx = 0.0f, efb = 0.0f;
-    uint32_t eemn = 0u, sehi = 0u;
+    uint32_t eemn = 0u, sehi = 0u, eneg = 0u;
     int ebR = 0;
     bool eok = true;
     if (em.w) {
@@ -391,10 +391,14 @@
                                                   ebR, eok);
                     wo[j] = wd;
                     sehi = max(sehi, word_sehi(wd));
+                    eneg |= wd;
                 }
             }
     }
-    if (em.w) wave_max_atomic(em.invalid + 5, sehi);
+    if (em.w) {
+        wave_max_atomic(em.invalid + 5, sehi);
+        wave_sign_record(em.invalid + 6, eneg);
+    }
     const bool ebad = em.w && !eok;
     if (__syncthreads_or(bad ? 1 : 0) && tid == 0) {
         atomicOr(gate, 1u);
diff --git a/fp8_quantization_amd/csrc/fp8approx.hip b/fp8_quantization_amd/csrc/fp8approx.hip
--- a/fp8_quantization_amd/csrc/fp8approx.hip
+++ b/fp8_quantization_amd/csrc/fp8approx.hip
@@ -83,7 +83,7 @@
     const int64_t MN = p.M * p.N;
     const float pb = post_bias(p);
     const EmitCtx ec = emit_ctx(p);
-    uint32_t sehi = 0;
+    uint32_t sehi = 0, neg = 0;
     const int S = p.splits;
     const bool vec = p.nchw ? ((p.hw & 3) == 0) : ((p.N & 3) == 0 && (p.ldc & 3) == 0);
     const bool aligned = ((((uintptr_t)p.C) & 15) == 0) && ((((uintptr_t)p.part) & 15) == 0) && ((MN & 3) == 0) &&
@@ -120,9 +120,12 @@
             }
             const float4 r = post4(p, o, acc, pb);
             *reinterpret_cast<float4 *>(p.C + o) = r;
-            if (p.em.w) emit4(p, ec, o, r, sehi);
-        }
-        if (p.em.w) wave_max_atomic(p.em.invalid + 5, sehi);
+            if (p.em.w) emit4(p, ec, o, r, sehi, neg);
+        }
+        if (p.em.w) {
+            wave_max_atomic(p.em.invalid + 5, sehi);
+            wave_sign_record(p.em.invalid + 6, neg);
+        }
         return;
     }
     for (int64_t q = (int64_t)blockIdx.x * blockDim.x + threadIdx.x; q < MN; q += stride) {
@@ -140,9 +143,12 @@
         }
         const float r = post1(p, o, epi(p.ep, p.ep_act, p.ep_lo, p.ep_hi, ch, acc), pb);
         p.C[o] = r;
-        if (p.em.w) emit1(p, ec, o, r, sehi);
-    }
-    if (p.em.w) wave_max_atomic(p.em.invalid + 5, sehi);
+        if (p.em.w) emit1(p, ec, o, r, sehi, neg);
+    }
+    if (p.em.w) {
+        wave_max_atomic(p.em.invalid + 5, sehi);
+        wave_sign_record(p.em.invalid + 6, neg);
+    }
 }
 
 __device__ __forceinline__ float load_A(const GemmArgs &p, int64_t m, int64_t k) {
@@ -191,9 +197,10 @@
             const float r = post1(p, o, epi(p.ep, p.ep_act, p.ep_lo, p.ep_hi, p.coff + n, s), post_bias(p));
             p.C[o] = r;
             if (p.em.w) {
-                uint32_t sh = 0;
-                emit1(p, emit_ctx(p), o, r, sh);
+                uint32_t sh = 0, ng = 0;
+                emit1(p, emit_ctx(p), o, r, sh, ng);
                 if (sh) atomicMax(p.em.invalid + 5, sh);
+                sign_record(p.em.invalid + 6, ng);
             }
         }
         return;
@@ -243,9 +250,10 @@
             const float r = post1(p, o, epi(p.ep, p.ep_act, p.ep_lo, p.ep_hi, p.coff + n, s[j] + part[j]), pb);
             p.C[o] = r;
             if (p.em.w) {
-                uint32_t sh = 0;
-                emit1(p, ec, o, r, sh);
+                uint32_t sh = 0, ng = 0;
+                emit1(p, ec, o, r, sh, ng);
                 if (sh) atomicMax(p.em.invalid + 5, sh);
+                sign_record(p.em.invalid + 6, ng);
             }
         }
     }
@@ -538,6 +546,7 @@
 }
 
 static int g_opt_xm_ncg = getenv("FP8A_XM_NCG") ? atoi(getenv("FP8A_XM_NCG")) : 0;
+static int g_opt_xm_sign_rows = getenv("FP8A_XM_SIGN_ROWS") ? atoi(getenv("FP8A_XM_SIGN_ROWS")) : 1;
 static int xm_ncg(int64_t N) {
     const int forced = g_opt_xm_ncg;
     if (forced == 1 || forced == 2 || forced == 4) return forced;
@@ -638,6 +647,7 @@
     return cache[dev];
 }
 
+static uint64_t g_splitk_launches = 0;
 static int choose_splits(int64_t M, int64_t N, int64_t K) {
     static int forced = -1;
     if (forced < 0) {
@@ -948,6 +958,7 @@
             a.wfmt = v5mx ? 4 : tt ? (tt16_form(a.Mw, a.ttf7, a.K) ? 2 : 1) : 0;
             if (a.wfmt == 1 && !g_opt_tt_band) a.ebr = nullptr;
             a.xncg = tt ? 4 : xm_ncg(a.N);
+            a.xm_signs = g_opt_xm_sign_rows;
             const bool use_img = a.in_img != nullptr && !tt && a.conv && a.fqin.mx != nullptr;
             if (use_img) a.aw = a.in_img + 64;
             a.af32 = !tt && !v5mx && !use_img && xm_af32(a) ? 1 : 0;
@@ -1010,6 +1021,7 @@
         const int64_t q = a.M * a.N;
         const unsigned rb = (unsigned)std::min<int64_t>((q / 4 + 255) / 256 + 1, 8192);
         splitk_reduce_kernel<<<rb, 256, 0, s>>>(a);
+        ++g_splitk_launches;
         rc = hip_check("fp8a split-K reduce launch");
         if (rc) return rc;
     }
@@ -1300,6 +1312,11 @@
         g_opt_xm_ncg = value;
         return old;
     }
+    if (strcmp(name, "xm_sign_rows") == 0) {
+        const int old = g_opt_xm_sign_rows;
+        g_opt_xm_sign_rows = value != 0;
+        return old;
+    }
     if (strcmp(name, "af32_maxct") == 0) {
         const int old = g_opt_af32_maxct;
         g_opt_af32_maxct = std::max(0, value);
@@ -1477,6 +1494,27 @@
         for (int i = 0; i < 3; ++i) v[i] += w[i];
     }
     for (int i = 0; i < 3; ++i) out[i] = v[i];
+    return FP8A_OK;
+}
+
+int fp8a_splitk_stats(uint64_t *out, int reset) {
+    if (out == nullptr) return fail(FP8A_EINVAL, "null pointer");
+    out[0] = g_splitk_launches;
+    if (reset) g_splitk_launches = 0;
+    return FP8A_OK;
+}
+
+int fp8a_xm_sign_stats(uint64_t *out, int reset) {
+    if (out == nullptr) return fail(FP8A_EINVAL, "null pointer");
+    if (hipDeviceSynchronize() != hipSuccess) return hip_check("fp8a_xm_sign_stats");
+    unsigned long long v[2] = {0, 0};
+    int (*parts[3])(unsigned long long *, bool) = {f8mx_signs_xf0, f8mx_signs_xf1, f8mx_signs_xf2};
+    for (auto f : parts) {
+        unsigned long long w[2] = {0, 0};
+        if (f(w, reset != 0) != 0) return hip_check("fp8a_xm_sign_stats");
+        for (int i = 0; i < 2; ++i) v[i] += w[i];
+    }
+    for (int i = 0; i < 2; ++i) out[i] = v[i];
     return FP8A_OK;
 }
 
@@ -1973,6 +2011,7 @@
     hdr[3] = (uint32_t)(128 - (int)fb) << 23;
     hdr[4] = (uint32_t)*bR;
     hdr[5] = 0u;
+    hdr[6] = 0u;
 }
 
 __global__ void word_image_fill_kernel(uint32_t *img, int64_t words) {
diff --git a/fp8_quantization_amd/csrc/fp8approx_common.h b/fp8_quantization_amd/csrc/fp8approx_common.h
--- a/fp8_quantization_amd/csrc/fp8approx_common.h
+++ b/fp8_quantization_amd/csrc/fp8approx_common.h
@@ -103,6 +103,7 @@
     int ttf7;
     int af32;
     int xncg;
+    int xm_signs;
     const uint2 *bqw;
     const uint32_t *lutw;
     const uint16_t *ebr;
@@ -248,22 +249,37 @@
 }
 __device__ __forceinline__ uint32_t word_sehi(uint32_t w) { return w == XM_ZERO_WORD ? 0u : 255u - (w >> 23); }
 
-__device__ __forceinline__ void emit1(const GemmArgs &p, const EmitCtx &e, int64_t o, float v, uint32_t &sehi) {
+constexpr uint32_t XM_SIGN_BIT = 0x40u;
+constexpr int XM_SIGN_W0 = 32, XM_SIGN_NW = 32;
+__device__ __forceinline__ void sign_record(uint32_t *dst, uint32_t words_or) {
+    if ((words_or & XM_SIGN_BIT) != 0u && __hip_atomic_load(dst, __ATOMIC_RELAXED, __HIP_MEMORY_SCOPE_AGENT) == 0u)
+        __hip_atomic_store(dst, 1u, __ATOMIC_RELAXED, __HIP_MEMORY_SCOPE_AGENT);
+}
+__device__ __forceinline__ void wave_sign_record(uint32_t *dst, uint32_t words_or) {
+    const bool any = __any((words_or & XM_SIGN_BIT) != 0u) != 0;
+    if ((threadIdx.x & 63) == 0 && any) sign_record(dst, XM_SIGN_BIT);
+}
+
+__device__ __forceinline__ void emit1(const GemmArgs &p, const EmitCtx &e, int64_t o, float v, uint32_t &sehi,
+                                      uint32_t &neg) {
     uint32_t wo;
     const uint32_t wi = emit_index(p, (uint32_t)o, wo);
     bool ok = true;
     const uint32_t w = emit_word(p, e, v, ok);
     p.em.w[wi] = w;
     sehi = max(sehi, word_sehi(w));
+    neg |= w;
     if (!ok) atomicOr(p.em.invalid, 1u);
 }
-__device__ __forceinline__ void emit4(const GemmArgs &p, const EmitCtx &e, int64_t o, float4 v, uint32_t &sehi) {
+__device__ __forceinline__ void emit4(const GemmArgs &p, const EmitCtx &e, int64_t o, float4 v, uint32_t &sehi,
+                                      uint32_t &neg) {
     uint32_t wo;
     const uint32_t wi = emit_index(p, (uint32_t)o, wo);
     bool ok0 = true, ok1 = true, ok2 = true, ok3 = true;
     const uint4 w = make_uint4(emit_word(p, e, v.x, ok0), emit_word(p, e, v.y, ok1), emit_word(p, e, v.z, ok2),
                                emit_word(p, e, v.w, ok3));
     sehi = max(max(sehi, max(word_sehi(w.x), word_sehi(w.y))), max(word_sehi(w.z), word_sehi(w.w)));
+    neg |= (w.x | w.y) | (w.z | w.w);
     if (wo + 3 < (uint32_t)p.em.Wo && (wi & 3u) == 0u) {
         *reinterpret_cast<uint4 *>(p.em.w + wi) = w;
     } else {
@@ -314,17 +330,17 @@
     const GemmArgs &q = p;
     const bool emit = EMIT && !partial && p.em.w != nullptr;
     const EmitCtx ec = EMIT ? emit_ctx(p) : EmitCtx{};
-    uint32_t sehi = 0;
+    uint32_t sehi = 0, neg = 0;
     auto fin1 = [&](int64_t o, float v) {
         if (partial) return v;
         v = post1<GELU>(q, o, v, pb);
-        if (emit) emit1(q, ec, o, v, sehi);
+        if (emit) emit1(q, ec, o, v, sehi, neg);
         return v;
     };
     auto fin4 = [&](int64_t o, float4 v) {
         if (partial) return v;
         v = post4<GELU>(q, o, v, pb);
-        if (emit) emit4(q, ec, o, v, sehi);
+        if (emit) emit4(q, ec, o, v, sehi, neg);
         return v;
     };
     if (!p.nchw) {
@@ -368,7 +384,10 @@
             }
         }
     }
-    if (emit) wave_max_atomic(p.em.invalid + 5, sehi);
-}
-
-}
+    if (emit) {
+        wave_max_atomic(p.em.invalid + 5, sehi);
+        wave_sign_record(p.em.invalid + 6, neg);
+    }
+}
+
+}
diff --git a/fp8_quantization_amd/csrc/fp8approx_launch.h b/fp8_quantization_amd/csrc/fp8approx_launch.h
--- a/fp8_quantization_amd/csrc/fp8approx_launch.h
+++ b/fp8_quantization_amd/csrc/fp8approx_launch.h
@@ -14,6 +14,9 @@
 int f8mx_clock_xf0(unsigned long long *v, bool reset);
 int f8mx_clock_xf1(unsigned long long *v, bool reset);
 int f8mx_clock_xf2(unsigned long long *v, bool reset);
+int f8mx_signs_xf0(unsigned long long *v, bool reset);
+int f8mx_signs_xf1(unsigned long long *v, bool reset);
+int f8mx_signs_xf2(unsigned long long *v, bool reset);
 
 void launch_tt(const GemmArgs &a, dim3 grid, hipStream_t s);
 int tt_rerun_stats(unsigned long long *v, bool reset);
diff --git a/fp8_quantization_amd/csrc/gemm_f8mx.h b/fp8_quantization_amd/csrc/gemm_f8mx.h
--- a/fp8_quantization_amd/csrc/gemm_f8mx.h
+++ b/fp8_quantization_amd/csrc/gemm_f8mx.h
@@ -154,6 +154,14 @@
 __device__ __forceinline__ void xm_record_se(const GemmArgs &p, uint32_t sehi) {
     if (p.Mw == 2 && p.wfmt == 0) wave_max_atomic(p.flag + 1, sehi);
 }
+__device__ __forceinline__ void xm_record_sign(const GemmArgs &p, uint32_t neg) {
+    if (p.wfmt != 0 || !p.xm_signs) return;
+    if (__syncthreads_or((neg & XM_SIGN_BIT) ? 1 : 0) && threadIdx.x == 0) {
+        uint32_t *w = p.flag + XM_SIGN_W0 + ((blockIdx.y * gridDim.x + blockIdx.x) & (XM_SIGN_NW - 1));
+        if (__hip_atomic_load(w, __ATOMIC_RELAXED, __HIP_MEMORY_SCOPE_WORKGROUP) == 0u)
+            __hip_atomic_store(w, 1u, __ATOMIC_RELAXED, __HIP_MEMORY_SCOPE_WORKGROUP);
+    }
+}
 
 #if FP8A_OWN_F8MX_DECODE
 __global__ __launch_bounds__(256) void xm_decode_a(const GemmArgs p) {
@@ -165,8 +173,10 @@
         *p.fq_ibias = bA;
     }
     if (p.gate != nullptr && __hip_atomic_load(p.gate, __ATOMIC_RELAXED, __HIP_MEMORY_SCOPE_AGENT) == 0u) {
-        if (p.Mw == 2 && p.wfmt == 0 && blockIdx.x == 0 && blockIdx.y == 0 && threadIdx.x == 0)
-            atomicMax(p.flag + 1, p.gate[5]);
+        if (p.wfmt == 0 && blockIdx.x == 0 && blockIdx.y == 0 && threadIdx.x == 0) {
+            if (p.Mw == 2) atomicMax(p.flag + 1, p.gate[5]);
+            if (p.xm_signs && p.gate[6] != 0u) atomicOr(p.flag + 3, 1u);
+        }
         return;
     }
     const uint32_t emnA = (uint32_t)(128 - bA) << 23;
@@ -177,6 +187,7 @@
     const int64_t hw = p.H * p.W;
     const int64_t rows = p.conv ? p.M / (p.Ho * p.Wo) : p.M, cols = p.conv ? p.aw_c * p.awH * p.awW : p.awld;
     uint32_t sehi = 0;
+    uint32_t neg = 0;
     const DFmt fv5 = dfmt(p.E, p.Mw, bA, false);
     auto word = [&](float v, bool &ok) {
         if (p.fqin.mx) v = fq_apply(v, fmx, fbias, p.fqin.M, p.fqin.S);
@@ -185,6 +196,7 @@
         if (p.wfmt) return tt_word_a(v, p.Mw, emnA, ok);
         const uint32_t w = xm_word_a(v, p.Mw, xm_xbias(p.Mw), emnA, bR, ok);
         sehi = max(sehi, word_sehi(w));
+        neg |= w;
         return w;
     };
     const uint32_t zw = p.wfmt ? 0u : XM_ZERO_WORD;
@@ -237,6 +249,7 @@
         if (__syncthreads_or(bad ? 1 : 0) && threadIdx.x == 0) atomicOr(p.flag, fb_bits(p, biasbad));
         if (__syncthreads_or(win ? 0 : 1) && threadIdx.x == 0) atomicOr(p.flag, 4u);
         xm_record_se(p, sehi);
+        xm_record_sign(p, neg);
         return;
     }
     const int64_t lim0 = p.conv ? cols : p.K, istride = p.conv ? p.Cin * hw : p.lda;
@@ -300,6 +313,7 @@
     if (__syncthreads_or(bad ? 1 : 0) && threadIdx.x == 0) atomicOr(p.flag, fb_bits(p, biasbad));
     if (__syncthreads_or(win ? 0 : 1) && threadIdx.x == 0) atomicOr(p.flag, 4u);
     xm_record_se(p, sehi);
+    xm_record_sign(p, neg);
 }
 #else
 __global__ void xm_decode_a(const GemmArgs p);
@@ -380,6 +394,7 @@
 #define FP8A_CLOCK_STAMP 0
 #endif
 __device__ unsigned long long g_clk[3];
+__device__ unsigned long long g_xm_sign[2];
 #if FP8A_CLOCK_STAMP
 #define FP8A_CLK_BEGIN const uint64_t clk_t0 = __builtin_amdgcn_s_memtime(), clk_r0 = __builtin_amdgcn_s_memrealtime();
 #define FP8A_CLK_END                                                                                   \
@@ -419,6 +434,11 @@
     const int64_t bid = (int64_t)blockIdx.x % tiles, split = (int64_t)blockIdx.x / tiles;
     const int64_t m0 = (bid % num_mt) * BMT;
     const int64_t n0 = (bid / num_mt) * BNT;
+    bool both = true;
+    if (!AF32 && p.xm_signs)
+        both = __any(__hip_atomic_load(p.flag + (lane < XM_SIGN_NW ? XM_SIGN_W0 + lane : 3), __ATOMIC_RELAXED,
+                                       __HIP_MEMORY_SCOPE_WORKGROUP) != 0u) != 0;
+    if (XF != 2 && blockIdx.x == 0 && tid == 0) atomicAdd(&g_xm_sign[both ? 1 : 0], 1ull);
     if (XF == 2 && !xm_half_gate(p, m0, BMT, n0, BNT)) return;
     const int kbeg = (int)(split * p.kchunk), kend = (int)min(p.K, (int64_t)kbeg + p.kchunk), K32 = (int)p.K;
     const int bR = *p.bR;
@@ -579,21 +599,37 @@
         for (int i = 0; i < APR; ++i)
             *reinterpret_cast<uint2 *>(&sm.aw[akp][2 * (arow + 64 * i)]) = make_uint2(wa[i][0], wa[i][1]);
         if (build) {
-#pragma unroll
-            for (int u = 0; u < BU; ++u) {
+            auto pk = [](uint32_t v, xm_u2 ad) { return __builtin_bit_cast(uint32_t, __builtin_bit_cast(xm_u2, v) + ad); };
+            auto unit_b = [&](int u) {
 #if XM_BDMA
-                const uint4 b = sm.bw[(bkk0 + u * BKU) * TXN + btx];
+                return sm.bw[(bkk0 + u * BKU) * TXN + btx];
 #else
-                const uint4 b = wbq[u];
-#endif
-                const uint2 s0 = *reinterpret_cast<const uint2 *>(lut + b.y + 8 * q4);
-                const uint2 s1 = *reinterpret_cast<const uint2 *>(lut + b.w + 8 * q4);
-                const xm_u2 a0 = __builtin_bit_cast(xm_u2, b.x), a1 = __builtin_bit_cast(xm_u2, b.z);
-                const xm_u2 n0 = __builtin_bit_cast(xm_u2, b.x ^ 0x80008000u), n1 = __builtin_bit_cast(xm_u2, b.z ^ 0x80008000u);
-                auto pk = [](uint32_t v, xm_u2 ad) { return __builtin_bit_cast(uint32_t, __builtin_bit_cast(xm_u2, v) + ad); };
-                uint32_t *d = &sm.tt[bkk0 + u * BKU][btx * 32 + q4 * 4];
-                *reinterpret_cast<uint4 *>(d) = make_uint4(pk(s0.x, a0), pk(s1.x, a1), pk(s0.y, a0), pk(s1.y, a1));
-                *reinterpret_cast<uint4 *>(d + 16) = make_uint4(pk(s0.x, n0), pk(s1.x, n1), pk(s0.y, n0), pk(s1.y, n1));
+                return wbq[u];
+#endif
+            };
+            if (both) {
+#pragma unroll
+                for (int u = 0; u < BU; ++u) {
+                    const uint4 b = unit_b(u);
+                    const uint2 s0 = *reinterpret_cast<const uint2 *>(lut + b.y + 8 * q4);
+                    const uint2 s1 = *reinterpret_cast<const uint2 *>(lut + b.w + 8 * q4);
+                    const xm_u2 a0 = __builtin_bit_cast(xm_u2, b.x), a1 = __builtin_bit_cast(xm_u2, b.z);
+                    const xm_u2 n0 = __builtin_bit_cast(xm_u2, b.x ^ 0x80008000u), n1 = __builtin_bit_cast(xm_u2, b.z ^ 0x80008000u);
+                    uint32_t *d = &sm.tt[bkk0 + u * BKU][btx * 32 + q4 * 4];
+                    *reinterpret_cast<uint4 *>(d) = make_uint4(pk(s0.x, a0), pk(s1.x, a1), pk(s0.y, a0), pk(s1.y, a1));
+                    *reinterpret_cast<uint4 *>(d + 16) = make_uint4(pk(s0.x, n0), pk(s1.x, n1), pk(s0.y, n0), pk(s1.y, n1));
+                }
+            } else {
+#pragma unroll
+                for (int u = 0; u < BU; ++u) {
+                    uint4 b = unit_b(u);
+                    asm volatile("" : "+v"(b.x), "+v"(b.z));
+                    const uint2 s0 = *reinterpret_cast<const uint2 *>(lut + b.y + 8 * q4);
+                    const uint2 s1 = *reinterpret_cast<const uint2 *>(lut + b.w + 8 * q4);
+                    const xm_u2 a0 = __builtin_bit_cast(xm_u2, b.x), a1 = __builtin_bit_cast(xm_u2, b.z);
+                    uint32_t *d = &sm.tt[bkk0 + u * BKU][btx * 32 + q4 * 4];
+                    *reinterpret_cast<uint4 *>(d) = make_uint4(pk(s0.x, a0), pk(s1.x, a1), pk(s0.y, a0), pk(s1.y, a1));
+                }
             }
         }
         __syncthreads();
diff --git a/fp8_quantization_amd/csrc/k_f8mx.hip b/fp8_quantization_amd/csrc/k_f8mx.hip
--- a/fp8_quantization_amd/csrc/k_f8mx.hip
+++ b/fp8_quantization_amd/csrc/k_f8mx.hip
@@ -44,15 +44,27 @@
     return 0;
 }
 
+static int signs_read(unsigned long long *v, bool reset) {
+    if (hipMemcpyFromSymbol(v, HIP_SYMBOL(g_xm_sign), 2 * sizeof(unsigned long long)) != hipSuccess) return -1;
+    if (reset) {
+        const unsigned long long z[2] = {0, 0};
+        if (hipMemcpyToSymbol(HIP_SYMBOL(g_xm_sign), z, sizeof(z)) != hipSuccess) return -1;
+    }
+    return 0;
+}
+
 #if FP8A_XF_PART == 0
 void launch_f8mx_xf0(const GemmArgs &a, hipStream_t s) { launch_xf<0>(a, s); }
 int f8mx_clock_xf0(unsigned long long *v, bool reset) { return clock_read(v, reset); }
+int f8mx_signs_xf0(unsigned long long *v, bool reset) { return signs_read(v, reset); }
 #elif FP8A_XF_PART == 1
 void launch_f8mx_xf1(const GemmArgs &a, hipStream_t s) { launch_xf<1>(a, s); }
 int f8mx_clock_xf1(unsigned long long *v, bool reset) { return clock_read(v, reset); }
+int f8mx_signs_xf1(unsigned long long *v, bool reset) { return signs_read(v, reset); }
 #else
 void launch_f8mx_xf2(const GemmArgs &a, hipStream_t s) { launch_xf<2>(a, s); }
 int f8mx_clock_xf2(unsigned long long *v, bool reset) { return clock_read(v, reset); }
+int f8mx_signs_xf2(unsigned long long *v, bool reset) { return signs_read(v, reset); }
 #endif
 
 }
diff --git a/include/fp8approx.h b/include/fp8approx.h
--- a/include/fp8approx.h
+++ b/include/fp8approx.h
@@ -31,6 +31,10 @@
 int fp8a_fallback_stats(uint64_t *out, int reset);
 
 int fp8a_path_stats(uint64_t *out, int reset);
+
+int fp8a_xm_sign_stats(uint64_t *out, int reset);
+
+int fp8a_splitk_stats(uint64_t *out, int reset);
 
 size_t fp8a_flag_arena_slot_bytes(fp8a_stream_t stream);
 
```
